# leeyevi/MV3D_TF

Measured on AMD Instinct MI355X. Metric: KITTI-shape frames/sec (RPN+3-view ROI-pool+NMS) at 1/2/4/8 MI355X, higher is better.
Workload: dtype f32

## Files before the change

### include/mv3d_hip.h

```cpp
#ifndef MV3D_HIP_H
#define MV3D_HIP_H
#include <stddef.h>
#include <stdint.h>
#ifdef __cplusplus
extern "C" {
#endif

typedef enum {
    MV3D_OK = 0,
    MV3D_ERR_INVALID_ARG = 1,
    MV3D_ERR_WORKSPACE = 2,
    MV3D_ERR_HIP = 3,
    MV3D_ERR_ZERO_DIVISION = 4
} mv3d_status;

int mv3d_version(void);
const char *mv3d_status_string(int status);


size_t mv3d_nms_workspace_bytes(int max_boxes);
int mv3d_nms_device(const float *dets_dev, int n, double thresh, int max_keep,
                    int32_t *keep_dev, int32_t *num_keep_dev, int32_t *status_dev,
                    void *workspace, size_t workspace_bytes, void *stream);

int mv3d_nms_round_plan(int num_boxes, int max_keep, int32_t *rounds_out);

int mv3d_nms_device_trace(const float *dets_dev, int n, double thresh, int max_keep,
                          int32_t *keep_dev, int32_t *num_keep_dev, int32_t *status_dev,
                          void *workspace, size_t workspace_bytes, void *stream, int64_t *trace_dev);

int mv3d_nms_host(int32_t *keep_out, int32_t *num_out, const float *dets_host, int n,
                  double thresh, int device_id);

void _nms(int *keep_out, int *num_out, const float *boxes_host, int boxes_num,
          int boxes_dim, float nms_overlap_thresh, int device_id);

typedef struct {
    int32_t feat_stride;
    int32_t pre_nms_topN;
    int32_t post_nms_topN;
    int32_t img_height;
    int32_t img_width;
    int32_t img_padding;
    int32_t nms_strict_gt;
    int32_t reserved0;
    double nms_thresh;
    double min_size;
} mv3d_proposal_params;

int mv3d_proposal_3d_capacity(int H, int W, const mv3d_proposal_params *p);
size_t mv3d_proposal_3d_workspace_bytes(int batch, int H, int W, const mv3d_proposal_params *p);
int mv3d_proposal_3d(const float *prob_dev, const float *pred_dev, int batch, int H, int W,
                     const float *im_info_dev, const float *calib_dev,
                     const mv3d_proposal_params *p,
                     float *blob_bv_dev, float *blob_img_dev, float *blob_3d_dev,
                     int32_t *num_out_dev, int32_t *status_dev,
                     void *workspace, size_t workspace_bytes, void *stream);
int mv3d_proposal_3d_masked(const float *prob_dev, const float *pred_dev, int batch, int H, int W,
                            const float *im_info_dev, const float *calib_dev,
                            const mv3d_proposal_params *p, const uint8_t *anchor_mask_dev,
                            float *blob_bv_dev, float *blob_img_dev, float *blob_3d_dev,
                            int32_t *num_out_dev, int32_t *status_dev,
                            void *workspace, size_t workspace_bytes, void *stream);

size_t mv3d_anchor_occupancy_workspace_bytes(int batch, int map_h, int map_w);
int mv3d_anchor_occupancy(const float *bev_dev, int batch, int map_h, int map_w, int channels,
                          int H, int W, int feat_stride, int min_cells,
                          uint8_t *mask_dev, int32_t *count_dev,
                          void *workspace, size_t workspace_bytes, void *stream);

int mv3d_roi_pool_forward(const float *bottom_data, float spatial_scale, int batch_size,
                          int num_rois, int height, int width, int channels,
                          int pooled_height, int pooled_width, const float *bottom_rois,
                          float *top_data, int32_t *argmax_data, void *stream);
int mv3d_roi_pool_backward(const float *top_diff, float spatial_scale, int batch_size,
                           int num_rois, int height, int width, int channels,
                           int pooled_height, int pooled_width, const float *bottom_rois,
                           float *bottom_diff, const int32_t *argmax_data, void *stream);

#define MV3D_MAX_ROI_VIEWS 4
typedef struct {
    const float *bottom_data;
    const float *bottom_rois;
    float *top_data;
    int32_t *argmax_data;
    float spatial_scale;
    int32_t batch_size, num_rois, height, width, channels;
} mv3d_roi_view;
int mv3d_roi_pool_forward_views(int num_views, const mv3d_roi_view *views, int pooled_height, int pooled_width,
                                void *stream);
int mv3d_roi_pool_forward_views_cold(int num_views, const mv3d_roi_view *views, int pooled_height, int pooled_width,
                                     void *stream);
int mv3d_roi_pool_forward_views_half(int num_views, const mv3d_roi_view *views, int pooled_height, int pooled_width,
                                     int top_type, int cold_maps, void *stream);

typedef struct {
    float *bottom_diff;
    const float *bottom_rois;
    const float *top_diff;
    const int32_t *argmax_data;
    float spatial_scale;
    int32_t batch_size, num_rois, height, width, channels;
} mv3d_roi_grad_view;
size_t mv3d_roi_pool_backward_workspace_bytes(int num_views, const mv3d_roi_grad_view *views, int pooled_height,
                                              int pooled_width);
int mv3d_roi_pool_backward_views(int num_views, const mv3d_roi_grad_view *views, int pooled_height, int pooled_width,
                                 void *workspace, size_t workspace_bytes, void *stream);
const char *mv3d_roi_pool_backward_path(int num_views, const mv3d_roi_grad_view *views, int pooled_height, int pooled_width,
                                        int have_workspace, int pair);

size_t mv3d_roi_pool_pair_workspace_bytes(int num_views, const mv3d_roi_grad_view *views, int pooled_height, int pooled_width);
int mv3d_roi_pool_forward_views_pair(int num_views, const mv3d_roi_view *views, int pooled_height, int pooled_width,
                                     int cold_maps, void *stream);
int mv3d_roi_pool_backward_views_pair(int num_views, const mv3d_roi_grad_view *views, int pooled_height, int pooled_width,
                                      void *workspace, size_t workspace_bytes, void *stream);
int mv3d_roi_pool_argmax_decode(int num_views, const mv3d_roi_view *views, int pooled_height, int pooled_width,
                                int32_t *const *argmax_out, void *stream);

int mv3d_ROIPoolForwardLaucher(const float *bottom_data, float spatial_scale, int num_rois, int height, int width, int channels,
                               int pooled_height, int pooled_width, const float *bottom_rois, float *top_data,
                               int32_t *argmax_data, void *stream);
int mv3d_ROIPoolBackwardLaucher(const float *top_diff, float spatial_scale, int batch_size, int num_rois, int height, int width,
                                int channels, int pooled_height, int pooled_width, const float *bottom_rois,
                                float *bottom_diff, const int32_t *argmax_data, void *stream);

int mv3d_rois_3d_to_fv(const float *rois_3d_dev, int num_rois, float *rois_fv_dev, void *stream);

#define MV3D_FV_MAX_FRAMES 1024
size_t mv3d_point_cloud_2_front_workspace(int num_frames);
int mv3d_point_cloud_2_front(const float *points_dev, const int32_t *offsets_dev, int num_frames, int total_points, float *fv_dev,
                             void *workspace_dev, void *stream);

typedef struct {
    int32_t feat_stride;
    int32_t clobber_positives;
    double negative_overlap;
    double positive_overlap;
} mv3d_anchor_target_params;

size_t mv3d_anchor_target_workspace_bytes(int H, int W, int G);
int mv3d_anchor_target_stage1(int H, int W, const float *im_info_dev, const float *gt_bv_dev,
                              const float *gt_3d_dev, int G, const mv3d_anchor_target_params *p,
                              float *labels_dev, float *targets_dev, int32_t *counts_dev,
                              uint8_t *fg_hi_dev, void *workspace, size_t workspace_bytes,
                              void *stream);
int mv3d_anchor_target_stage2(int H, int W, const mv3d_anchor_target_params *p,
                              const int32_t *disable_fg_dev, int n_dis_fg,
                              const int32_t *disable_bg1_dev, int n_dis_bg1,
                              const int32_t *disable_bg2_dev, int n_dis_bg2,
                              float *labels_dev, float *anchors_dev, float *anchors_3d_dev,
                              int32_t *n_anchors_dev, int anchors_cap,
                              void *workspace, size_t workspace_bytes, void *stream);

int mv3d_anchor_target_stage1_batch(int batch, int H, int W, const float *im_info_dev, const float *const *gt_bv_dev,
                                    const float *const *gt_3d_dev, const int *G, const mv3d_anchor_target_params *p,
                                    float *labels_dev, float *targets_dev, int32_t *const *counts_dev,
                                    uint8_t *const *fg_hi_dev, void *const *workspace, size_t workspace_bytes, void *stream);
int mv3d_anchor_target_stage1_batch_masked(int batch, int H, int W, const float *im_info_dev, const float *const *gt_bv_dev,
                                           const float *const *gt_3d_dev, const int *G, const mv3d_anchor_target_params *p,
                                           const uint8_t *const *anchor_mask_dev, float *labels_dev, float *targets_dev,
                                           int32_t *const *counts_dev, uint8_t *const *fg_hi_dev, void *const *workspace,
                                           size_t workspace_bytes, void *stream);
int mv3d_anchor_target_stage2_batch(int batch, int H, int W, const mv3d_anchor_target_params *p,
                                    const int32_t *const *disable_fg_dev, const int *n_dis_fg,
                                    const int32_t *const *disable_bg1_dev, const int *n_dis_bg1,
                                    const int32_t *const *disable_bg2_dev, const int *n_dis_bg2, float *labels_dev,
                                    float *anchors_dev, float *anchors_3d_dev, int32_t *n_anchors_dev, int anchors_cap,
                                    void *const *workspace, size_t workspace_bytes, void *stream);

typedef struct {
    int32_t num_classes;
    int32_t frame_index;
    double fg_thresh;
    double bg_thresh_hi;
    double bg_thresh_lo;
} mv3d_proposal_target_params;

size_t mv3d_proposal_target_workspace_bytes(int num_rois, int G);
int mv3d_proposal_target_stage1(const float *rois_bv_dev, const float *rois_3d_dev, int num_rois,
                                const float *gt_bv_dev, const float *gt_3d_dev, int G,
                                const mv3d_proposal_target_params *p, int32_t *counts_dev,
                                void *workspace, size_t workspace_bytes, void *stream);
int mv3d_proposal_target_stage2(const float *rois_bv_dev, const float *rois_3d_dev, int num_rois,
                                const float *gt_bv_dev, const float *gt_3d_dev,
                                const float *gt_corners_dev, int G, const float *calib_dev,
                                const mv3d_proposal_target_params *p,
                                const int32_t *fg_pick_dev, int n_fg, const int32_t *bg_pick_dev, int n_bg,
                                float *rois_bv_out, float *rois_img_out, int32_t *labels_out,
                                float *bbox_targets_out, float *rois_3d_out,
                                void *workspace, size_t workspace_bytes, void *stream);

int mv3d_proposal_target_stage1_batch(int batch, const float *const *rois_bv_dev, const float *const *rois_3d_dev,
                                      const int *num_rois, const float *const *gt_bv_dev, const float *const *gt_3d_dev,
                                      const int *G, const mv3d_proposal_target_params *params, int32_t *const *counts_dev,
                                      void *const *workspace, const size_t *workspace_bytes, void *stream);
int mv3d_proposal_target_stage2_batch(int batch, const float *const *rois_bv_dev, const float *const *rois_3d_dev,
                                      const int *num_rois, const float *const *gt_bv_dev, const float *const *gt_3d_dev,
                                      const float *const *gt_corners_dev, const int *G, const float *const *calib_dev,
                                      const mv3d_proposal_target_params *params, const int32_t *const *fg_pick_dev,
                                      const int *n_fg, const int32_t *const *bg_pick_dev, const int *n_bg,
                                      float *const *rois_bv_out, float *const *rois_img_out, int32_t *const *labels_out,
                                      float *const *bbox_targets_out, float *const *rois_3d_out, float *const *rois_fv_out,
                                      void *const *workspace, const size_t *workspace_bytes, void *stream);
int mv3d_proposal_target_stage1_batch_devn(int batch, const float *const *rois_bv_dev, const float *const *rois_3d_dev,
                                           const int *num_rois_cap, const int32_t *const *num_rois_dev,
                                           const float *const *gt_bv_dev, const float *const *gt_3d_dev, const int *G,
                                           const mv3d_proposal_target_params *params, int32_t *const *counts_dev,
                                           void *const *workspace, const size_t *workspace_bytes, void *stream);
int mv3d_proposal_target_stage2_batch_devn(int batch, const float *const *rois_bv_dev, const float *const *rois_3d_dev,
                                           const int *num_rois_cap, const int32_t *const *num_rois_dev,
                                           const float *const *gt_bv_dev, const float *const *gt_3d_dev,
                                           const float *const *gt_corners_dev, const int *G, const float *const *calib_dev,
                                           const mv3d_proposal_target_params *params, const int32_t *const *fg_pick_dev,
                                           const int *n_fg, const int32_t *const *bg_pick_dev, const int *n_bg,
                                           float *const *rois_bv_out, float *const *rois_img_out, int32_t *const *labels_out,
                                           float *const *bbox_targets_out, float *const *rois_3d_out, float *const *rois_fv_out,
                                           void *const *workspace, const size_t *workspace_bytes, void *stream);

int mv3d_point_cloud_2_top(const float *points_dev, int num_points, float *top_dev, void *stream);

int mv3d_point_cloud_2_top_shape(double res, double zres, double side_lo, double side_hi, double fwd_lo, double fwd_hi,
                                 double height_lo, double height_hi, int *dims);
int mv3d_point_cloud_2_top_ranges(const float *points_dev, int num_points, double res, double zres, double side_lo, double side_hi,
                                  double fwd_lo, double fwd_hi, double height_lo, double height_hi, float *top_dev,
                                  int *status_dev, void *stream);

int mv3d_point_cloud_2_top_batch(const float *points_dev, const int32_t *offsets_dev, int num_frames, int total_points,
                                 const double *ranges8_host, float *top_dev, int32_t *status_dev, void *stream);
int mv3d_point_cloud_2_top_batch_dense(const float *points_dev, const int32_t *offsets_dev, int num_frames, int total_points,
                                       const double *ranges8_host, float *top_dev, int32_t *status_dev, void *stream);

int mv3d_point_cloud_2_top_paper_batch(const float *points_dev, const int32_t *offsets_dev, int num_frames, int total_points,
                                       const double *ranges8_host, float *top_dev, void *workspace_dev, int32_t *status_dev,
                                       void *stream);
size_t mv3d_point_cloud_2_top_paper_workspace(int num_frames, const double *ranges8_host);
int mv3d_point_cloud_2_top_paper_shape(double res, double zres, double side_lo, double side_hi, double fwd_lo, double fwd_hi,
                                       double height_lo, double height_hi, int *dims);
int mv3d_bev_density_table(float *out64);

size_t mv3d_scan_crop_workspace(int total_points);
int mv3d_scan_crop_tile_rows(void);
int mv3d_scan_crop_to_image(const float *points_dev, const int32_t *offsets_dev, int num_frames, int total_points,
                            const float *calib_dev, const int32_t *image_hw_dev, float *points_out_dev, int32_t *offsets_out_dev,
                            void *workspace_dev, size_t workspace_bytes, void *stream);

int mv3d_scan_transform(const float *points_dev, const int32_t *offsets_dev, int num_frames, int total_points,
                        const double *xform_dev, float *points_out_dev, void *stream);

int mv3d_legacy_permutation(void *mt19937_state, int32_t n, int32_t *out);
typedef struct {
    int32_t n_fg, n_bg, n_low;
    int32_t pt_n_fg, pt_n_bg;
    int32_t reserved0;
    const uint8_t *fg_alive;
} mv3d_draw_frame;
typedef struct {
    int32_t rpn_batchsize;
    int32_t rpn_num_fg;
    int32_t rois_per_image;
    int32_t roi_fg_max;
} mv3d_draw_params;
int mv3d_draw_training_subsamples(void *mt19937_state, int batch, const mv3d_draw_frame *frames, const mv3d_draw_params *par,
                                  int32_t *lists, size_t lists_cap, int32_t *sizes, int32_t *scratch, size_t scratch_cap);

typedef struct {
    int32_t batch, H, W, num_classes;
    int32_t proposal_cap;
    int32_t anchor_cap;
    int32_t roi_cap;
    int32_t max_gt;
    mv3d_proposal_params proposal;
    mv3d_anchor_target_params anchor;
    mv3d_proposal_target_params target;
    mv3d_draw_params draw;
} mv3d_train_path_config;
typedef struct {
    float *blob_bv, *blob_img, *blob_3d;
    int32_t *num_proposals;
    void *proposal_ws; size_t proposal_ws_bytes;
    float *rpn_labels, *rpn_targets;
    float *anchors, *anchors_3d;
    int32_t *n_anchors;
    uint8_t *report; size_t report_row;
    int32_t *pt_counts;
    void *anchor_ws; size_t anchor_ws_bytes;
    void *target_ws; size_t target_ws_bytes;
    float *rois_bev, *rois_rgb, *rois_fv;
    float *rois_3d; int32_t *labels; float *bbox_targets;
    int32_t *lists; size_t lists_cap;
    uint8_t *h_report; size_t h_report_row;
    int32_t *h_pt_counts;
    int32_t *h_num_proposals;
    int32_t *h_lists;
    int32_t *h_scratch; size_t scratch_cap;
} mv3d_train_path_slot;
typedef struct mv3d_train_path mv3d_train_path;
int mv3d_train_path_create(const mv3d_train_path_config *config, int depth, const mv3d_train_path_slot *slots, int helper_thread,
                           mv3d_train_path **out);
int mv3d_train_path_configure(mv3d_train_path *path, const mv3d_train_path_config *config);
int mv3d_train_path_submit(mv3d_train_path *path, int slot, const float *prob_dev, const float *pred_dev, const float *im_info_dev,
                           const float *calib_dev, const float *const *gt_bv_dev, const float *const *gt_3d_dev,
                           const float *const *gt_corners_dev, const int *G, void *mt19937_state, void *stream);
int mv3d_train_path_submit_masked(mv3d_train_path *path, int slot, const float *prob_dev, const float *pred_dev,
                                  const float *im_info_dev, const float *calib_dev, const float *const *gt_bv_dev,
                                  const float *const *gt_3d_dev, const float *const *gt_corners_dev, const int *G,
                                  const uint8_t *anchor_mask_dev, void *mt19937_state, void *stream);
int mv3d_train_path_finish(mv3d_train_path *path, int slot, int32_t *rows_out, int32_t *num_proposals_out, int32_t *sizes_out);
int mv3d_train_path_host_seconds(mv3d_train_path *path, double *wait_s, double *draw_s);
void mv3d_train_path_destroy(mv3d_train_path *path);

int mv3d_gt_encode(const float *box_cam_dev, const double *cos_sin_dev, int num_objects, const float *inv_rot_dev,
                   const float *tr_velo_to_cam_dev, float *corners_cam_dev, float *corners_lidar_dev,
                   float *boxes_3d_dev, float *boxes_bv_dev, void *stream);

int mv3d_box_detect_tail(const float *rois_3d_dev, const float *bbox_pred_dev, int num_rois, int num_classes,
                         float *corners_dev, float *pred_cnr_r_dev, float *pred_bv_dev, float *pred_bv_r_dev,
                         void *stream);

typedef struct {
    int32_t num_classes;
    int32_t rows_per_frame;
    int32_t max_per_image;
    int32_t nms_strict_gt;
    float score_thresh;
    int32_t reserved0;
    double nms_thresh;
} mv3d_detect_post_params;

size_t mv3d_detect_post_workspace_bytes(int batch, const mv3d_detect_post_params *p);
int mv3d_detect_post(const float *cls_prob_dev, const float *pred_bv_dev, const float *corners_dev,
                     const float *pred_cnr_r_dev, const int32_t *num_rois_dev, int batch,
                     const mv3d_detect_post_params *p, float *det_bv_dev, float *det_cnr_dev, float *det_cnr_r_dev,
                     int32_t *det_row_dev, int32_t *det_count_dev, int32_t *status_dev, void *workspace,
                     size_t workspace_bytes, void *stream);

#define MV3D_DETECT_STATUS_NONFINITE 2
size_t mv3d_detect_post_oriented_workspace_bytes(int batch, const mv3d_detect_post_params *p);
int mv3d_detect_post_oriented(const float *cls_prob_dev, const float *pred_bv_dev, const float *corners_dev,
                              const float *pred_cnr_r_dev, const int32_t *num_rois_dev, int batch,
                              const mv3d_detect_post_params *p, int footprint_source, float *det_bv_dev, float *det_cnr_dev,
                              float *det_cnr_r_dev, int32_t *det_row_dev, int32_t *det_count_dev, int32_t *status_dev,
                              void *workspace, size_t workspace_bytes, void *stream);

size_t mv3d_loss_workspace_bytes(int rows);
int mv3d_rpn_loss(const float *rpn_cls_score_dev, const float *rpn_labels_dev, const float *rpn_bbox_pred_dev,
                  const float *rpn_bbox_targets_dev, int num_anchors, float sigma, float *losses_dev,
                  float *d_cls_score_dev, float *d_bbox_pred_dev, void *workspace, size_t workspace_bytes, void *stream);
int mv3d_rcnn_loss(const float *cls_score_dev, const int32_t *labels_dev, const float *bbox_pred_dev,
                   const float *bbox_targets_dev, int num_rois, int num_classes, int box_dim, float sigma,
                   float *losses_dev, float *d_cls_score_dev, float *d_bbox_pred_dev, void *workspace,
                   size_t workspace_bytes, void *stream);
int mv3d_rcnn_loss_ignore(const float *cls_score_dev, const int32_t *labels_dev, const float *bbox_pred_dev,
                          const float *bbox_targets_dev, int num_rois, int num_classes, int box_dim, float sigma,
                          float *losses_dev, float *d_cls_score_dev, float *d_bbox_pred_dev, void *workspace,
                          size_t workspace_bytes, void *stream);

int mv3d_ignore_relabel(const float *rpn_labels_dev, const int32_t *roi_labels_dev, const float *rois_bv_dev,
                        const float *rois_img_dev, int num_rois, const float *calib_dev, int batch, int H, int W,
                        int feat_stride, const float *ignore_bv_dev, const int32_t *ignore_bv_off_dev, int ignore_bv_rows,
                        const float *ignore_img_dev, const int32_t *ignore_img_off_dev, int ignore_img_rows, double overlap,
                        float *rpn_labels_out_dev, int32_t *roi_labels_out_dev, int32_t *counts_dev, int32_t *status_dev,
                        void *stream);

int mv3d_conv3x3_f16(const void *x_framed, const void *w_packed, const float *bias, void *y, int batch, int height, int width,
                     int c_in, int c_out, int out_framed, int out_f32, int relu, void *stream);
int mv3d_conv3x3_f32(const void *x_framed, const void *w_packed, const float *bias, void *y, int batch, int height, int width, int c_in,
                     int c_out, int out_framed, int relu, void *stream);
int mv3d_maxpool2x2_f32(const void *x_framed, void *y_framed, int batch, int height, int width, int channels, void *stream);
int mv3d_frame_nhwc_f32(const float *x_nhwc, void *y_framed, int batch, int height, int width, int channels, int channels_out,
                        void *stream);
int mv3d_conv3x3_bf16(const void *x_framed, const void *w_packed, const float *bias, void *y, int batch, int height, int width,
                      int c_in, int c_out, int out_framed, int out_f32, int relu, void *stream);
int mv3d_conv3x3_gated_bf16(const void *x_framed, const void *w_packed, const float *bias, const void *gate_framed, void *y,
                            int batch, int height, int width, int c_in, int c_out, void *stream);
int mv3d_maxpool2x2_bf16(const void *x_framed, void *y_framed, int batch, int height, int width, int channels, void *stream);
int mv3d_frame_nhwc_bf16(const float *x_nhwc, void *y_framed, int batch, int height, int width, int channels, int channels_out,
                         void *stream);
int mv3d_maxpool2x2_bwd_bf16(const void *y_framed, const void *g_pooled_framed, void *gy_framed, int batch, int height, int width,
                             int channels, void *stream);
int mv3d_maxpool2x2_bwd_f32(const void *y_framed, const void *g_pooled_framed, void *gy_framed, int batch, int height, int width,
                            int channels, void *stream);
#define MV3D_MAX_CONV_VIEWS 3
typedef struct {
    const void *x_framed;
    const void *w_packed;
    const float *bias;
    const void *gate_framed;
    void *y;
    int32_t batch, height, width, reserved0;
} mv3d_conv_view;
int mv3d_conv3x3_views_f16(int num_views, const mv3d_conv_view *views, int c_in, int c_out, int out_framed, int out_f32, int relu,
                           void *stream);
int mv3d_conv3x3_views_bf16(int num_views, const mv3d_conv_view *views, int c_in, int c_out, int out_framed, int out_f32, int relu,
                            void *stream);
int mv3d_conv3x3_views_f32(int num_views, const mv3d_conv_view *views, int c_in, int c_out, int out_framed, int relu, void *stream);
int mv3d_conv3x3_pool_views_f16(int num_views, const mv3d_conv_view *views, int c_in, int c_out, void *stream);
int mv3d_conv3x3_pool_views_bf16(int num_views, const mv3d_conv_view *views, int c_in, int c_out, void *stream);
const char *mv3d_conv3x3_path(int operand_bytes, int num_views, const int32_t *pixels, int c_in, int c_out, int out_f32, int gated,
                              int pool);
typedef struct {
    const void *x_framed;
    const void *g_pooled_framed;
    void *y_framed;
    int32_t batch, height, width, reserved0;
} mv3d_pool_view;
int mv3d_maxpool2x2_views_f16(int num_views, const mv3d_pool_view *views, int channels, void *stream);
int mv3d_maxpool2x2_views_bf16(int num_views, const mv3d_pool_view *views, int channels, void *stream);
int mv3d_maxpool2x2_views_f32(int num_views, const mv3d_pool_view *views, int channels, void *stream);
int mv3d_maxpool2x2_bwd_views_bf16(int num_views, const mv3d_pool_view *views, int channels, void *stream);
int mv3d_maxpool2x2_bwd_views_f32(int num_views, const mv3d_pool_view *views, int channels, void *stream);
size_t mv3d_conv3x3_wgrad_workspace_bytes(int batch, int height, int width, int c_in, int c_out);
int mv3d_conv3x3_wgrad_bf16(const void *x_framed, const void *dy_framed, float *dw, float *db, int batch, int height, int width,
                            int c_in, int c_in_real, int c_out, void *workspace, size_t workspace_bytes, void *stream);
size_t mv3d_conv3x3_wgrad_f32_workspace_bytes(int batch, int height, int width, int c_in, int c_out);
int mv3d_conv3x3_wgrad_f32(const void *x_framed, const void *dy_framed, float *dw, float *db, int batch, int height, int width,
                           int c_in, int c_in_real, int c_out, void *workspace, size_t workspace_bytes, void *stream);
typedef struct {
    const void *x_framed;
    const void *dy_framed;
    float *dw;
    float *db;
    int32_t batch, height, width;
    int32_t c_in_real;
} mv3d_wgrad_view;
size_t mv3d_conv3x3_wgrad_views_workspace_bytes(int num_views, const mv3d_wgrad_view *views, int c_in, int c_out, int f32_maps);
int mv3d_conv3x3_wgrad_views_bf16(int num_views, const mv3d_wgrad_view *views, int c_in, int c_in_real, int c_out, void *workspace,
                                  size_t workspace_bytes, void *stream);
int mv3d_conv3x3_wgrad_views_f32(int num_views, const mv3d_wgrad_view *views, int c_in, int c_in_real, int c_out, void *workspace,
                                 size_t workspace_bytes, void *stream);
int mv3d_conv3x3_pack_bf16(const float *w_oihw, void *fwd_packed, void *dgrad_packed, int c_out, int c_in, int c_in_pad, void *stream);
typedef struct {
    const float *w_oihw;
    void *fwd_packed, *dgrad_packed;
    int32_t c_out, c_in, c_in_pad, reserved0;
} mv3d_pack_item;
int mv3d_conv3x3_pack_many_bf16(int num_items, const mv3d_pack_item *items, void *stream);
int mv3d_conv3x3_pack_many_f32(int num_items, const mv3d_pack_item *items, void *stream);
int mv3d_maxpool2x2_f16(const void *x_framed, void *y_framed, int batch, int height, int width, int channels, void *stream);
int mv3d_frame_nhwc_f16(const float *x_nhwc, void *y_framed, int batch, int height, int width, int channels, int channels_out,
                        void *stream);

int mv3d_softmax_rows(const float *logits_dev, float *prob_dev, long long rows, int classes, void *stream);

typedef struct {
    float *param;
    const float *grad;
    float *exp_avg, *exp_avg_sq;
    long long numel;
    void *param_lowp;
} mv3d_adam_tensor;
int mv3d_adam_chunk_elements(void);
int mv3d_adam_step(const mv3d_adam_tensor *tensors_dev, const int32_t *chunk_tensor_dev, const int32_t *chunk_first_dev, int num_chunks,
                   double lr, double beta1, double beta2, double eps, int step, int lowp_dtype ,
                   void *stream);

#define MV3D_KITTI_MAX_DETS 2048
#define MV3D_KITTI_NUM_SAMPLE_PTS 41
typedef struct {
    int32_t num_frames, num_dets, num_gts, img_height;
    const int32_t *det_off, *gt_off;
    const int32_t *offsets_dev;
    const float *det_cnr_dev, *det_score_dev, *calib_dev, *gt_cnr_dev;
    const int32_t *gt_cls_dev;
    const float *gt_attr_dev;
} mv3d_kitti_split;
int mv3d_kitti_eval_overlaps(const mv3d_kitti_split *split, long long num_pairs, double *iou_dev, double *det_height_dev,
                             void *stream);
int mv3d_kitti_eval_match(const mv3d_kitti_split *split, long long num_pairs, const double *iou_dev, const double *det_height_dev,
                          int eval_class, int neighbor_class, double min_overlap, float *matched_dev, void *stream);
int mv3d_kitti_eval_count(const mv3d_kitti_split *split, long long num_pairs, const double *iou_dev, const double *det_height_dev,
                          int eval_class, int neighbor_class, double min_overlap, const float *thresholds_dev,
                          const int32_t *num_thresholds_dev, int32_t *counts_dev, void *stream);

typedef struct {
    int32_t num_dontcare, reserved0;
    const int32_t *dc_off;
    const int32_t *dc_off_dev;
    const float *gt_box_dev, *gt_alpha_dev, *dc_box_dev;
    const int32_t *image_shape_dev;
} mv3d_kitti_image_split;
int mv3d_kitti_eval_image_boxes(const mv3d_kitti_split *split, const mv3d_kitti_image_split *image, double *det_box_dev,
                                double *det_cam_dev, void *stream);
int mv3d_kitti_eval_match_2d(const mv3d_kitti_split *split, const mv3d_kitti_image_split *image, const double *det_box_dev,
                             int eval_class, int neighbor_class, double min_overlap, float *matched_dev, void *stream);
int mv3d_kitti_eval_count_2d(const mv3d_kitti_split *split, const mv3d_kitti_image_split *image, const double *det_box_dev,
                             const double *det_cam_dev, int eval_class, int neighbor_class, double min_overlap,
                             const float *thresholds_dev, const int32_t *num_thresholds_dev, int32_t *counts_dev,
                             double *similarity_dev, void *stream);

#define MV3D_RECALL_MAX_GT 256
#define MV3D_RECALL_SHORT_ASSERT 0
#define MV3D_RECALL_SHORT_ZERO 1
#define MV3D_RECALL_STATUS_SHORT 1
#define MV3D_RECALL_STATUS_NONFINITE 2
typedef struct {
    int32_t num_frames, num_gts, num_limits, num_thresholds, short_mode, reserved0;
    long long num_boxes;
    const int32_t *box_off, *gt_off;
    const int32_t *box_off_dev, *gt_off_dev;
    const float *boxes_dev, *gt_dev;
    const int32_t *limits_dev;
    const double *thresholds_dev;
} mv3d_recall_split;
int mv3d_proposal_recall(const mv3d_recall_split *split, double *gt_overlaps_dev, int32_t *counts_dev, int32_t *status_dev,
                         void *stream);

#define MV3D_RECALL3D_BOX6 0
#define MV3D_RECALL3D_CNR24 1
typedef struct {
    int32_t num_frames, num_gts, num_limits, num_thresholds, short_mode, box_format;
    long long num_boxes, num_pairs;
    const int32_t *box_off, *gt_off, *pair_off;
    const int32_t *box_off_dev, *gt_off_dev, *pair_off_dev;
    const float *boxes_dev, *gt_cnr_dev;
    const int32_t *limits_dev;
    const double *thresholds_dev;
} mv3d_recall3d_split;
size_t mv3d_proposal_recall_3d_workspace_bytes(long long num_pairs);
int mv3d_proposal_recall_3d(const mv3d_recall3d_split *split, double *iou_ws_dev, double *gt_overlaps_dev, int32_t *counts_dev,
                            int32_t *status_dev, void *stream);
int mv3d_proposal_recall_3d_overlaps(const mv3d_recall3d_split *split, double *iou_ws_dev, int32_t *status_dev, void *stream);
int mv3d_proposal_recall_3d_match(const mv3d_recall3d_split *split, const double *iou_ws_dev, double *gt_overlaps_dev,
                                  int32_t *counts_dev, int32_t *status_dev, void *stream);

int mv3d_mirror_columns(float *data_dev, long long rows, int width, int channels, void *stream);

#define MV3D_IMAGE_MAX_FRAMES 1024
int mv3d_image_blob(const uint8_t *pixels_dev, int total_bytes, const int32_t *frames_dev, int num_frames, const double *means3_host,
                    int canvas_h, int canvas_w, float *out_dev, void *stream);

int mv3d_fusion_join_forward(const void *h_dev, int dtype, int sets_in, int paths, int views, int rows, int channels,
                             const uint8_t *keep, const uint8_t *drop_dev, float scale, void *out_dev, void *stream);
int mv3d_fusion_join_backward(const void *h_dev, const void *g_out_dev, int dtype, int sets_in, int paths, int views, int rows,
                              int channels, const uint8_t *keep, const uint8_t *drop_dev, float scale, void *g_h_dev, void *stream);

typedef struct {
    const void *in;
    void *out;
    int64_t frame_stride, row_stride, pixel_stride;
    int32_t dtype, batch, height, width, channels, factor;
} mv3d_upsample_view;
int mv3d_upsample_bilinear_views(int num_views, const mv3d_upsample_view *views, void *stream);
int mv3d_upsample_bilinear_backward_views(int num_views, const mv3d_upsample_view *views, void *stream);

#ifdef __cplusplus
}
#endif
#endif
```

### mv3d_tf_amd/_lib.py

```python
import ctypes as C
import os

import torch

_HERE = os.path.dirname(os.path.abspath(__file__))
LIB_PATH = os.path.join(_HERE, "libmv3d_hip.so")

OK, ERR_INVALID_ARG, ERR_WORKSPACE, ERR_HIP, ERR_ZERO_DIVISION = 0, 1, 2, 3, 4
MAX_ROI_VIEWS = 4


class ProposalParams(C.Structure):
    _fields_ = [("feat_stride", C.c_int32), ("pre_nms_topN", C.c_int32), ("post_nms_topN", C.c_int32),
                ("img_height", C.c_int32), ("img_width", C.c_int32), ("img_padding", C.c_int32),
                ("nms_strict_gt", C.c_int32), ("reserved0", C.c_int32), ("nms_thresh", C.c_double), ("min_size", C.c_double)]


class DetectPostParams(C.Structure):
    _fields_ = [("num_classes", C.c_int32), ("rows_per_frame", C.c_int32), ("max_per_image", C.c_int32),
                ("nms_strict_gt", C.c_int32), ("score_thresh", C.c_float), ("reserved0", C.c_int32), ("nms_thresh", C.c_double)]


class AnchorTargetParams(C.Structure):
    _fields_ = [("feat_stride", C.c_int32), ("clobber_positives", C.c_int32),
                ("negative_overlap", C.c_double), ("positive_overlap", C.c_double)]


class RoiView(C.Structure):
    _fields_ = [("bottom_data", C.c_void_p), ("bottom_rois", C.c_void_p), ("top_data", C.c_void_p),
                ("argmax_data", C.c_void_p), ("spatial_scale", C.c_float), ("batch_size", C.c_int32),
                ("num_rois", C.c_int32), ("height", C.c_int32), ("width", C.c_int32), ("channels", C.c_int32)]


class RoiGradView(C.Structure):
    _fields_ = [("bottom_diff", C.c_void_p), ("bottom_rois", C.c_void_p), ("top_diff", C.c_void_p),
                ("argmax_data", C.c_void_p), ("spatial_scale", C.c_float), ("batch_size", C.c_int32),
                ("num_rois", C.c_int32), ("height", C.c_int32), ("width", C.c_int32), ("channels", C.c_int32)]


class ProposalTargetParams(C.Structure):
    _fields_ = [("num_classes", C.c_int32), ("frame_index", C.c_int32), ("fg_thresh", C.c_double),
                ("bg_thresh_hi", C.c_double), ("bg_thresh_lo", C.c_double)]


class DrawFrame(C.Structure):
    _fields_ = [("n_fg", C.c_int32), ("n_bg", C.c_int32), ("n_low", C.c_int32), ("pt_n_fg", C.c_int32), ("pt_n_bg", C.c_int32),
                ("reserved0", C.c_int32), ("fg_alive", C.c_void_p)]


class DrawParams(C.Structure):
    _fields_ = [("rpn_batchsize", C.c_int32), ("rpn_num_fg", C.c_int32), ("rois_per_image", C.c_int32), ("roi_fg_max", C.c_int32)]


class TrainPathConfig(C.Structure):
    _fields_ = [("batch", C.c_int32), ("H", C.c_int32), ("W", C.c_int32), ("num_classes", C.c_int32), ("proposal_cap", C.c_int32),
                ("anchor_cap", C.c_int32), ("roi_cap", C.c_int32), ("max_gt", C.c_int32), ("proposal", ProposalParams),
                ("anchor", AnchorTargetParams), ("target", ProposalTargetParams), ("draw", DrawParams)]


class TrainPathSlot(C.Structure):
    _fields_ = [("blob_bv", C.c_void_p), ("blob_img", C.c_void_p), ("blob_3d", C.c_void_p), ("num_proposals", C.c_void_p),
                ("proposal_ws", C.c_void_p), ("proposal_ws_bytes", C.c_size_t), ("rpn_labels", C.c_void_p), ("rpn_targets", C.c_void_p),
                ("anchors", C.c_void_p), ("anchors_3d", C.c_void_p), ("n_anchors", C.c_void_p), ("report", C.c_void_p),
                ("report_row", C.c_size_t), ("pt_counts", C.c_void_p), ("anchor_ws", C.c_void_p), ("anchor_ws_bytes", C.c_size_t),
                ("target_ws", C.c_void_p), ("target_ws_bytes", C.c_size_t), ("rois_bev", C.c_void_p), ("rois_rgb", C.c_void_p),
                ("rois_fv", C.c_void_p), ("rois_3d", C.c_void_p), ("labels", C.c_void_p), ("bbox_targets", C.c_void_p),
                ("lists", C.c_void_p), ("lists_cap", C.c_size_t), ("h_report", C.c_void_p), ("h_report_row", C.c_size_t),
                ("h_pt_counts", C.c_void_p), ("h_num_proposals", C.c_void_p), ("h_lists", C.c_void_p), ("h_scratch", C.c_void_p),
                ("scratch_cap", C.c_size_t)]


class ConvView(C.Structure):
    _fields_ = [("x_framed", C.c_void_p), ("w_packed", C.c_void_p), ("bias", C.c_void_p), ("gate_framed", C.c_void_p), ("y", C.c_void_p),
                ("batch", C.c_int32), ("height", C.c_int32), ("width", C.c_int32), ("reserved0", C.c_int32)]


class PoolView(C.Structure):
    _fields_ = [("x_framed", C.c_void_p), ("g_pooled_framed", C.c_void_p), ("y_framed", C.c_void_p),
                ("batch", C.c_int32), ("height", C.c_int32), ("width", C.c_int32), ("reserved0", C.c_int32)]


class WgradView(C.Structure):
    _fields_ = [("x_framed", C.c_void_p), ("dy_framed", C.c_void_p), ("dw", C.c_void_p), ("db", C.c_void_p),
                ("batch", C.c_int32), ("height", C.c_int32), ("width", C.c_int32), ("c_in_real", C.c_int32)]


class PackItem(C.Structure):
    _fields_ = [("w_oihw", C.c_void_p), ("fwd_packed", C.c_void_p), ("dgrad_packed", C.c_void_p),
                ("c_out", C.c_int32), ("c_in", C.c_int32), ("c_in_pad", C.c_int32), ("reserved0", C.c_int32)]


class AdamTensor(C.Structure):
    _fields_ = [("param", C.c_void_p), ("grad", C.c_void_p), ("exp_avg", C.c_void_p), ("exp_avg_sq", C.c_void_p), ("numel", C.c_longlong),
                ("param_lowp", C.c_void_p)]


class KittiSplit(C.Structure):
    _fields_ = [("num_frames", C.c_int32), ("num_dets", C.c_int32), ("num_gts", C.c_int32), ("img_height", C.c_int32),
                ("det_off", C.c_void_p), ("gt_off", C.c_void_p), ("offsets_dev", C.c_void_p), ("det_cnr_dev", C.c_void_p),
                ("det_score_dev", C.c_void_p), ("calib_dev", C.c_void_p), ("gt_cnr_dev", C.c_void_p), ("gt_cls_dev", C.c_void_p),
                ("gt_attr_dev", C.c_void_p)]


class KittiImageSplit(C.Structure):
    _fields_ = [("num_dontcare", C.c_int32), ("reserved0", C.c_int32), ("dc_off", C.c_void_p), ("dc_off_dev", C.c_void_p),
                ("gt_box_dev", C.c_void_p), ("gt_alpha_dev", C.c_void_p), ("dc_box_dev", C.c_void_p), ("image_shape_dev", C.c_void_p)]


class RecallSplit(C.Structure):
    _fields_ = [("num_frames", C.c_int32), ("num_gts", C.c_int32), ("num_limits", C.c_int32), ("num_thresholds", C.c_int32),
                ("short_mode", C.c_int32), ("reserved0", C.c_int32), ("num_boxes", C.c_longlong), ("box_off", C.c_void_p),
                ("gt_off", C.c_void_p), ("box_off_dev", C.c_void_p), ("gt_off_dev", C.c_void_p), ("boxes_dev", C.c_void_p),
                ("gt_dev", C.c_void_p), ("limits_dev", C.c_void_p), ("thresholds_dev", C.c_void_p)]


class Recall3dSplit(C.Structure):
    _fields_ = [("num_frames", C.c_int32), ("num_gts", C.c_int32), ("num_limits", C.c_int32), ("num_thresholds", C.c_int32),
                ("short_mode", C.c_int32), ("box_format", C.c_int32), ("num_boxes", C.c_longlong), ("num_pairs", C.c_longlong),
                ("box_off", C.c_void_p), ("gt_off", C.c_void_p), ("pair_off", C.c_void_p), ("box_off_dev", C.c_void_p),
                ("gt_off_dev", C.c_void_p), ("pair_off_dev", C.c_void_p), ("boxes_dev", C.c_void_p), ("gt_cnr_dev", C.c_void_p),
                ("limits_dev", C.c_void_p), ("thresholds_dev", C.c_void_p)]


class UpsampleView(C.Structure):
    _fields_ = [("in_", C.c_void_p), ("out", C.c_void_p), ("frame_stride", C.c_int64), ("row_stride", C.c_int64),
                ("pixel_stride", C.c_int64), ("dtype", C.c_int32), ("batch", C.c_int32), ("height", C.c_int32), ("width", C.c_int32),
                ("channels", C.c_int32), ("factor", C.c_int32)]


_P = C.c_void_p
_SIGS = {
    "mv3d_version": (C.c_int, []),
    "mv3d_status_string": (C.c_char_p, [C.c_int]),
    "mv3d_nms_workspace_bytes": (C.c_size_t, [C.c_int]),
    "mv3d_nms_round_plan": (C.c_int, [C.c_int, C.c_int, C.POINTER(C.c_int32)]),
    "mv3d_nms_device": (C.c_int, [_P, C.c_int, C.c_double, C.c_int, _P, _P, _P, _P, C.c_size_t, _P]),
    "mv3d_nms_device_trace": (C.c_int, [_P, C.c_int, C.c_double, C.c_int, _P, _P, _P, _P, C.c_size_t, _P, _P]),
    "mv3d_nms_host": (C.c_int, [_P, _P, _P, C.c_int, C.c_double, C.c_int]),
    "_nms": (None, [_P, _P, _P, C.c_int, C.c_int, C.c_float, C.c_int]),
    "mv3d_proposal_3d_capacity": (C.c_int, [C.c_int, C.c_int, C.POINTER(ProposalParams)]),
    "mv3d_proposal_3d_workspace_bytes": (C.c_size_t, [C.c_int, C.c_int, C.c_int, C.POINTER(ProposalParams)]),
    "mv3d_proposal_3d": (C.c_int, [_P, _P, C.c_int, C.c_int, C.c_int, _P, _P, C.POINTER(ProposalParams),
                                   _P, _P, _P, _P, _P, _P, C.c_size_t, _P]),
    "mv3d_proposal_3d_masked": (C.c_int, [_P, _P, C.c_int, C.c_int, C.c_int, _P, _P, C.POINTER(ProposalParams),
                                          _P, _P, _P, _P, _P, _P, _P, C.c_size_t, _P]),
    "mv3d_anchor_occupancy_workspace_bytes": (C.c_size_t, [C.c_int, C.c_int, C.c_int]),
    "mv3d_anchor_occupancy": (C.c_int, [_P, C.c_int, C.c_int, C.c_int, C.c_int, C.c_int, C.c_int, C.c_int, C.c_int, _P, _P, _P,
                                        C.c_size_t, _P]),
    "mv3d_roi_pool_forward": (C.c_int, [_P, C.c_float, C.c_int, C.c_int, C.c_int, C.c_int, C.c_int, C.c_int,
                                        C.c_int, _P, _P, _P, _P]),
    "mv3d_roi_pool_backward": (C.c_int, [_P, C.c_float, C.c_int, C.c_int, C.c_int, C.c_int, C.c_int, C.c_int,
                                         C.c_int, _P, _P, _P, _P]),
    "mv3d_anchor_target_workspace_bytes": (C.c_size_t, [C.c_int, C.c_int, C.c_int]),
    "mv3d_anchor_target_stage1": (C.c_int, [C.c_int, C.c_int, _P, _P, _P, C.c_int, C.POINTER(AnchorTargetParams),
                                            _P, _P, _P, _P, _P, C.c_size_t, _P]),
    "mv3d_anchor_target_stage2": (C.c_int, [C.c_int, C.c_int, C.POINTER(AnchorTargetParams), _P, C.c_int, _P,
                                            C.c_int, _P, C.c_int, _P, _P, _P, _P, C.c_int, _P, C.c_size_t, _P]),
    "mv3d_anchor_target_stage1_batch": (C.c_int, [C.c_int, C.c_int, C.c_int, _P, _P, _P, _P, C.POINTER(AnchorTargetParams), _P, _P, _P, _P,
                                                  _P, C.c_size_t, _P]),
    "mv3d_anchor_target_stage1_batch_masked": (C.c_int, [C.c_int, C.c_int, C.c_int, _P, _P, _P, _P, C.POINTER(AnchorTargetParams), _P, _P,
                                                         _P, _P, _P, _P, C.c_size_t, _P]),
    "mv3d_anchor_target_stage2_batch": (C.c_int, [C.c_int, C.c_int, C.c_int, C.POINTER(AnchorTargetParams), _P, _P, _P, _P, _P, _P, _P,
                                                  _P, _P, _P, C.c_int, _P, C.c_size_t, _P]),
    "mv3d_proposal_target_stage1_batch": (C.c_int, [C.c_int, _P, _P, _P, _P, _P, _P, _P, _P, _P, _P, _P]),
    "mv3d_proposal_target_stage2_batch": (C.c_int, [C.c_int, _P, _P, _P, _P, _P, _P, _P, _P, _P, _P, _P, _P, _P, _P, _P, _P, _P, _P, _P,
                                                    _P, _P, _P]),
    "mv3d_proposal_target_stage1_batch_devn": (C.c_int, [C.c_int, _P, _P, _P, _P, _P, _P, _P, _P, _P, _P, _P, _P]),
    "mv3d_proposal_target_stage2_batch_devn": (C.c_int, [C.c_int, _P, _P, _P, _P, _P, _P, _P, _P, _P, _P, _P, _P, _P, _P, _P, _P, _P, _P,
                                                         _P, _P, _P, _P, _P]),
    "mv3d_proposal_target_workspace_bytes": (C.c_size_t, [C.c_int, C.c_int]),
    "mv3d_proposal_target_stage1": (C.c_int, [_P, _P, C.c_int, _P, _P, C.c_int, C.POINTER(ProposalTargetParams), _P, _P,
                                              C.c_size_t, _P]),
    "mv3d_proposal_target_stage2": (C.c_int, [_P, _P, C.c_int, _P, _P, _P, C.c_int, _P, C.POINTER(ProposalTargetParams),
                                              _P, C.c_int, _P, C.c_int, _P, _P, _P, _P, _P, _P, C.c_size_t, _P]),
    "mv3d_point_cloud_2_top": (C.c_int, [_P, C.c_int, _P, _P]),
    "mv3d_point_cloud_2_top_shape": (C.c_int, [C.c_double] * 8 + [_P]),
    "mv3d_point_cloud_2_top_ranges": (C.c_int, [_P, C.c_int] + [C.c_double] * 8 + [_P, _P, _P]),
    "mv3d_point_cloud_2_top_batch": (C.c_int, [_P, _P, C.c_int, C.c_int, _P, _P, _P, _P]),
    "mv3d_point_cloud_2_top_batch_dense": (C.c_int, [_P, _P, C.c_int, C.c_int, _P, _P, _P, _P]),
    "mv3d_point_cloud_2_top_paper_batch": (C.c_int, [_P, _P, C.c_int, C.c_int, _P, _P, _P, _P, _P]),
    "mv3d_point_cloud_2_top_paper_workspace": (C.c_size_t, [C.c_int, _P]),
    "mv3d_point_cloud_2_top_paper_shape": (C.c_int, [C.c_double] * 8 + [_P]),
    "mv3d_bev_density_table": (C.c_int, [_P]),
    "mv3d_scan_crop_workspace": (C.c_size_t, [C.c_int]),
    "mv3d_scan_crop_tile_rows": (C.c_int, []),
    "mv3d_scan_crop_to_image": (C.c_int, [_P, _P, C.c_int, C.c_int, _P, _P, _P, _P, _P, C.c_size_t, _P]),
    "mv3d_scan_transform": (C.c_int, [_P, _P, C.c_int, C.c_int, _P, _P, _P]),
    "mv3d_box_detect_tail": (C.c_int, [_P, _P, C.c_int, C.c_int, _P, _P, _P, _P, _P]),
    "mv3d_detect_post_workspace_bytes": (C.c_size_t, [C.c_int, C.POINTER(DetectPostParams)]),
    "mv3d_detect_post": (C.c_int, [_P, _P, _P, _P, _P, C.c_int, C.POINTER(DetectPostParams), _P, _P, _P, _P, _P, _P, _P, C.c_size_t,
                                   _P]),
    "mv3d_detect_post_oriented_workspace_bytes": (C.c_size_t, [C.c_int, C.POINTER(DetectPostParams)]),
    "mv3d_detect_post_oriented": (C.c_int, [_P, _P, _P, _P, _P, C.c_int, C.POINTER(DetectPostParams), C.c_int, _P, _P, _P, _P, _P, _P,
                                            _P, C.c_size_t, _P]),
    "mv3d_loss_workspace_bytes": (C.c_size_t, [C.c_int]),
    "mv3d_rpn_loss": (C.c_int, [_P, _P, _P, _P, C.c_int, C.c_float, _P, _P, _P, _P, C.c_size_t, _P]),
    "mv3d_rcnn_loss": (C.c_int, [_P, _P, _P, _P, C.c_int, C.c_int, C.c_int, C.c_float, _P, _P, _P, _P, C.c_size_t, _P]),
    "mv3d_rcnn_loss_ignore": (C.c_int, [_P, _P, _P, _P, C.c_int, C.c_int, C.c_int, C.c_float, _P, _P, _P, _P, C.c_size_t, _P]),
    "mv3d_ignore_relabel": (C.c_int, [_P, _P, _P, _P, C.c_int, _P, C.c_int, C.c_int, C.c_int, C.c_int, _P, _P, C.c_int, _P, _P, C.c_int,
                                      C.c_double, _P, _P, _P, _P, _P]),
    "mv3d_roi_pool_forward_views": (C.c_int, [C.c_int, C.POINTER(RoiView), C.c_int, C.c_int, _P]),
    "mv3d_roi_pool_forward_views_cold": (C.c_int, [C.c_int, C.POINTER(RoiView), C.c_int, C.c_int, _P]),
    "mv3d_roi_pool_forward_views_half": (C.c_int, [C.c_int, C.POINTER(RoiView), C.c_int, C.c_int, C.c_int, C.c_int, _P]),
    "mv3d_roi_pool_backward_workspace_bytes": (C.c_size_t, [C.c_int, C.POINTER(RoiGradView), C.c_int, C.c_int]),
    "mv3d_roi_pool_backward_views": (C.c_int, [C.c_int, C.POINTER(RoiGradView), C.c_int, C.c_int, _P, C.c_size_t, _P]),
    "mv3d_roi_pool_backward_path": (C.c_char_p, [C.c_int, C.POINTER(RoiGradView), C.c_int, C.c_int, C.c_int, C.c_int]),
    "mv3d_roi_pool_pair_workspace_bytes": (C.c_size_t, [C.c_int, C.POINTER(RoiGradView), C.c_int, C.c_int]),
    "mv3d_roi_pool_forward_views_pair": (C.c_int, [C.c_int, C.POINTER(RoiView), C.c_int, C.c_int, C.c_int, _P]),
    "mv3d_roi_pool_backward_views_pair": (C.c_int, [C.c_int, C.POINTER(RoiGradView), C.c_int, C.c_int, _P, C.c_size_t, _P]),
    "mv3d_roi_pool_argmax_decode": (C.c_int, [C.c_int, C.POINTER(RoiView), C.c_int, C.c_int, C.POINTER(C.c_void_p), _P]),
    "mv3d_ROIPoolForwardLaucher": (C.c_int, [_P, C.c_float, C.c_int, C.c_int, C.c_int, C.c_int, C.c_int, C.c_int, _P, _P, _P, _P]),
    "mv3d_ROIPoolBackwardLaucher": (C.c_int, [_P, C.c_float, C.c_int, C.c_int, C.c_int, C.c_int, C.c_int, C.c_int, C.c_int, _P, _P, _P, _P]),
    "mv3d_rois_3d_to_fv": (C.c_int, [_P, C.c_int, _P, _P]),
    "mv3d_point_cloud_2_front_workspace": (C.c_size_t, [C.c_int]),
    "mv3d_point_cloud_2_front": (C.c_int, [_P, _P, C.c_int, C.c_int, _P, _P, _P]),
    "mv3d_legacy_permutation": (C.c_int, [_P, C.c_int32, _P]),
    "mv3d_draw_training_subsamples": (C.c_int, [_P, C.c_int, C.POINTER(DrawFrame), C.POINTER(DrawParams), _P, C.c_size_t, _P, _P,
                                                C.c_size_t]),
    "mv3d_train_path_create": (C.c_int, [C.POINTER(TrainPathConfig), C.c_int, C.POINTER(TrainPathSlot), C.c_int, C.POINTER(C.c_void_p)]),
    "mv3d_train_path_configure": (C.c_int, [_P, C.POINTER(TrainPathConfig)]),
    "mv3d_train_path_submit": (C.c_int, [_P, C.c_int, _P, _P, _P, _P, _P, _P, _P, _P, _P, _P]),
    "mv3d_train_path_submit_masked": (C.c_int, [_P, C.c_int, _P, _P, _P, _P, _P, _P, _P, _P, _P, _P, _P]),
    "mv3d_train_path_finish": (C.c_int, [_P, C.c_int, _P, _P, _P]),
    "mv3d_train_path_host_seconds": (C.c_int, [_P, C.POINTER(C.c_double), C.POINTER(C.c_double)]),
    "mv3d_train_path_destroy": (None, [_P]),
    "mv3d_gt_encode": (C.c_int, [_P, _P, C.c_int, _P, _P, _P, _P, _P, _P, _P]),
    "mv3d_conv3x3_f16": (C.c_int, [_P, _P, _P, _P, C.c_int, C.c_int, C.c_int, C.c_int, C.c_int, C.c_int, C.c_int, C.c_int, _P]),
    "mv3d_conv3x3_f32": (C.c_int, [_P, _P, _P, _P, C.c_int, C.c_int, C.c_int, C.c_int, C.c_int, C.c_int, C.c_int, _P]),
    "mv3d_maxpool2x2_f32": (C.c_int, [_P, _P, C.c_int, C.c_int, C.c_int, C.c_int, _P]),
    "mv3d_frame_nhwc_f32": (C.c_int, [_P, _P, C.c_int, C.c_int, C.c_int, C.c_int, C.c_int, _P]),
    "mv3d_conv3x3_bf16": (C.c_int, [_P, _P, _P, _P, C.c_int, C.c_int, C.c_int, C.c_int, C.c_int, C.c_int, C.c_int, C.c_int, _P]),
    "mv3d_maxpool2x2_bf16": (C.c_int, [_P, _P, C.c_int, C.c_int, C.c_int, C.c_int, _P]),
    "mv3d_frame_nhwc_bf16": (C.c_int, [_P, _P, C.c_int, C.c_int, C.c_int, C.c_int, C.c_int, _P]),
    "mv3d_conv3x3_wgrad_workspace_bytes": (C.c_size_t, [C.c_int, C.c_int, C.c_int, C.c_int, C.c_int]),
    "mv3d_conv3x3_wgrad_bf16": (C.c_int, [_P, _P, _P, _P, C.c_int, C.c_int, C.c_int, C.c_int, C.c_int, C.c_int, _P, C.c_size_t, _P]),
    "mv3d_conv3x3_wgrad_f32_workspace_bytes": (C.c_size_t, [C.c_int, C.c_int, C.c_int, C.c_int, C.c_int]),
    "mv3d_conv3x3_wgrad_f32": (C.c_int, [_P, _P, _P, _P, C.c_int, C.c_int, C.c_int, C.c_int, C.c_int, C.c_int, _P, C.c_size_t, _P]),
    "mv3d_conv3x3_pack_bf16": (C.c_int, [_P, _P, _P, C.c_int, C.c_int, C.c_int, _P]),
    "mv3d_conv3x3_gated_bf16": (C.c_int, [_P, _P, _P, _P, _P, C.c_int, C.c_int, C.c_int, C.c_int, C.c_int, _P]),
    "mv3d_maxpool2x2_bwd_f32": (C.c_int, [_P, _P, _P, C.c_int, C.c_int, C.c_int, C.c_int, _P]),
    "mv3d_maxpool2x2_bwd_bf16": (C.c_int, [_P, _P, _P, C.c_int, C.c_int, C.c_int, C.c_int, _P]),
    "mv3d_conv3x3_views_f16": (C.c_int, [C.c_int, C.POINTER(ConvView), C.c_int, C.c_int, C.c_int, C.c_int, C.c_int, _P]),
    "mv3d_conv3x3_views_bf16": (C.c_int, [C.c_int, C.POINTER(ConvView), C.c_int, C.c_int, C.c_int, C.c_int, C.c_int, _P]),
    "mv3d_conv3x3_views_f32": (C.c_int, [C.c_int, C.POINTER(ConvView), C.c_int, C.c_int, C.c_int, C.c_int, _P]),
    "mv3d_conv3x3_pool_views_f16": (C.c_int, [C.c_int, C.POINTER(ConvView), C.c_int, C.c_int, _P]),
    "mv3d_conv3x3_pool_views_bf16": (C.c_int, [C.c_int, C.POINTER(ConvView), C.c_int, C.c_int, _P]),
    "mv3d_conv3x3_path": (C.c_char_p, [C.c_int, C.c_int, C.POINTER(C.c_int32), C.c_int, C.c_int, C.c_int, C.c_int, C.c_int]),
    "mv3d_maxpool2x2_views_f16": (C.c_int, [C.c_int, C.POINTER(PoolView), C.c_int, _P]),
    "mv3d_maxpool2x2_views_bf16": (C.c_int, [C.c_int, C.POINTER(PoolView), C.c_int, _P]),
    "mv3d_maxpool2x2_views_f32": (C.c_int, [C.c_int, C.POINTER(PoolView), C.c_int, _P]),
    "mv3d_maxpool2x2_bwd_views_bf16": (C.c_int, [C.c_int, C.POINTER(PoolView), C.c_int, _P]),
    "mv3d_maxpool2x2_bwd_views_f32": (C.c_int, [C.c_int, C.POINTER(PoolView), C.c_int, _P]),
    "mv3d_conv3x3_wgrad_views_workspace_bytes": (C.c_size_t, [C.c_int, C.POINTER(WgradView), C.c_int, C.c_int, C.c_int]),
    "mv3d_conv3x3_wgrad_views_bf16": (C.c_int, [C.c_int, C.POINTER(WgradView), C.c_int, C.c_int, C.c_int, _P, C.c_size_t, _P]),
    "mv3d_conv3x3_wgrad_views_f32": (C.c_int, [C.c_int, C.POINTER(WgradView), C.c_int, C.c_int, C.c_int, _P, C.c_size_t, _P]),
    "mv3d_conv3x3_pack_many_bf16": (C.c_int, [C.c_int, C.POINTER(PackItem), _P]),
    "mv3d_conv3x3_pack_many_f32": (C.c_int, [C.c_int, C.POINTER(PackItem), _P]),
    "mv3d_maxpool2x2_f16": (C.c_int, [_P, _P, C.c_int, C.c_int, C.c_int, C.c_int, _P]),
    "mv3d_frame_nhwc_f16": (C.c_int, [_P, _P, C.c_int, C.c_int, C.c_int, C.c_int, C.c_int, _P]),
    "mv3d_softmax_rows": (C.c_int, [_P, _P, C.c_longlong, C.c_int, _P]),
    "mv3d_adam_chunk_elements": (C.c_int, []),
    "mv3d_adam_step": (C.c_int, [_P, _P, _P, C.c_int, C.c_double, C.c_double, C.c_double, C.c_double, C.c_int, C.c_int, _P]),
    "mv3d_kitti_eval_overlaps": (C.c_int, [C.POINTER(KittiSplit), C.c_longlong, _P, _P, _P]),
    "mv3d_kitti_eval_match": (C.c_int, [C.POINTER(KittiSplit), C.c_longlong, _P, _P, C.c_int, C.c_int, C.c_double, _P, _P]),
    "mv3d_kitti_eval_count": (C.c_int, [C.POINTER(KittiSplit), C.c_longlong, _P, _P, C.c_int, C.c_int, C.c_double, _P, _P, _P, _P]),
    "mv3d_kitti_eval_image_boxes": (C.c_int, [C.POINTER(KittiSplit), C.POINTER(KittiImageSplit), _P, _P, _P]),
    "mv3d_kitti_eval_match_2d": (C.c_int, [C.POINTER(KittiSplit), C.POINTER(KittiImageSplit), _P, C.c_int, C.c_int, C.c_double, _P,
                                           _P]),
    "mv3d_kitti_eval_count_2d": (C.c_int, [C.POINTER(KittiSplit), C.POINTER(KittiImageSplit), _P, _P, C.c_int, C.c_int, C.c_double,
                                           _P, _P, _P, _P, _P]),
    "mv3d_proposal_recall": (C.c_int, [C.POINTER(RecallSplit), _P, _P, _P, _P]),
    "mv3d_proposal_recall_3d_workspace_bytes": (C.c_size_t, [C.c_longlong]),
    "mv3d_proposal_recall_3d": (C.c_int, [C.POINTER(Recall3dSplit), _P, _P, _P, _P, _P]),
    "mv3d_proposal_recall_3d_overlaps": (C.c_int, [C.POINTER(Recall3dSplit), _P, _P, _P]),
    "mv3d_proposal_recall_3d_match": (C.c_int, [C.POINTER(Recall3dSplit), _P, _P, _P, _P, _P]),
    "mv3d_mirror_columns": (C.c_int, [_P, C.c_longlong, C.c_int, C.c_int, _P]),
    "mv3d_image_blob": (C.c_int, [_P, C.c_int, _P, C.c_int, C.POINTER(C.c_double), C.c_int, C.c_int, _P, _P]),
    "mv3d_fusion_join_forward": (C.c_int, [_P, C.c_int, C.c_int, C.c_int, C.c_int, C.c_int, C.c_int, _P, _P, C.c_float, _P, _P]),
    "mv3d_fusion_join_backward": (C.c_int, [_P, _P, C.c_int, C.c_int, C.c_int, C.c_int, C.c_int, C.c_int, _P, _P, C.c_float, _P, _P]),
    "mv3d_upsample_bilinear_views": (C.c_int, [C.c_int, C.POINTER(UpsampleView), _P]),
    "mv3d_upsample_bilinear_backward_views": (C.c_int, [C.c_int, C.POINTER(UpsampleView), _P]),
}
EXPORTS = tuple(_SIGS)

_lib = None


def lib():
    global _lib
    if _lib is None:
        if not os.path.exists(LIB_PATH):
            raise RuntimeError(
                f"{LIB_PATH} is missing: the HIP extension is the product and has no fallback. "
                "Build it with `python -m mv3d_tf_amd.build` (or __graft_entry__.build()).")
        handle = C.CDLL(LIB_PATH)
        for name, (res, args) in _SIGS.items():
            fn = getattr(handle, name)
            fn.restype = res
            fn.argtypes = args
        _lib = handle
    return _lib


class Mv3dError(RuntimeError):
    def __init__(self, status, where):
        self.status = status
        super().__init__(f"{where}: {lib().mv3d_status_string(status).decode()} (status {status})")


def check(status, where):
    if status == ERR_ZERO_DIVISION:
        raise ZeroDivisionError("float division")
    if status != OK:
        raise Mv3dError(status, where)
```

### mv3d_tf_amd/csrc/anchor_target.hip

```cpp
#include <math.h>
#include "geometry.h"

__device__ __forceinline__ double mv3d_log(double x)
{
    if (x != x || x < 0) return NAN;
    if (x == 0) return -INFINITY;
    if (isinf(x)) return x;
    int k;
    double m = frexp(x, &k);
    if (m < 0.70710678118654752440) { m *= 2.0; k -= 1; }
    const double s = (m - 1.0) / (m + 1.0);
    const double z = s * s;
    double p = 1.0 / 39;
#pragma unroll
    for (int d = 37; d >= 1; d -= 2) p = fma(p, z, 1.0 / d);
    const double LN2_HI = 6.93147180369123816490e-01, LN2_LO = 1.90821492927058770002e-10;
    const double lm = 2.0 * s * p;
    return fma((double)k, LN2_HI, fma((double)k, LN2_LO, lm));
}

struct AtDev {
    int H, W, N, G, stride, clobber;
    double neg_ov, pos_ov;
    const float *im_info, *gt_bv, *gt_3d;
    const uint8_t *mask;
    double *max_ov;
    int32_t *argmax;
    unsigned long long *gtpart;
    int nblk;
    float *labels, *targets;
};

#define AT_MAX_BATCH 16
struct AtLists {
    int32_t *fg, *bg, *low;
};
struct AtFrame {
    AtDev d;
    AtLists lists;
    int32_t *counts;
    uint8_t *fg_hi;
    int32_t *agg1, *agg2;
    const int32_t *dis_fg, *dis_bg1, *dis_bg2;
    int n_dis_fg, n_dis_bg1, n_dis_bg2;
    float *anchors, *anchors_3d;
    int32_t *n_anchors;
};
struct AtBatch { AtFrame f[AT_MAX_BATCH]; int cap, n_agg1, n_agg2; };

__device__ __forceinline__ bool anchor_box(const AtDev &d, int n, int &x1, int &y1, int &x2, int &y2)
{
    grid_anchor(n, d.W, d.stride, x1, y1, x2, y2);
    return x1 >= 0 && y1 >= 0 && (double)x2 < (double)d.im_info[1] && (double)y2 < (double)d.im_info[0] && (!d.mask || d.mask[n]);
}

__global__ __launch_bounds__(256) void at_overlap_kernel(AtBatch bt)
{
    const AtDev &d = bt.f[blockIdx.y].d;
    if (blockIdx.x == 0) {
        const AtFrame &F = bt.f[blockIdx.y];
        for (int t = threadIdx.x; t < bt.n_agg1; t += blockDim.x) F.agg1[t] = 0;
        for (int t = threadIdx.x; t < bt.n_agg2; t += blockDim.x) F.agg2[t] = 0;
    }
    __shared__ float s_gt[TARGET_MAX_GT * 4];
    __shared__ unsigned long long s_max[TARGET_MAX_GT];
    stage_gt_bv(d.gt_bv, d.G, s_gt);
    for (int g = threadIdx.x; g < d.G; g += blockDim.x) s_max[g] = 0ull;
    __syncthreads();
    const int n = blockIdx.x * blockDim.x + threadIdx.x;
    if (n < d.N) {
        int x1, y1, x2, y2;
        const bool inside = anchor_box(d, n, x1, y1, x2, y2);
        double mx = -1.0;
        int am = 0;
        if (inside) {
            for (int g = 0; g < d.G; ++g) {
                const double o = bbox_overlap_f64(x1, y1, x2, y2, s_gt[4 * g], s_gt[4 * g + 1], s_gt[4 * g + 2], s_gt[4 * g + 3]);
                if (o > mx) { mx = o; am = g; }
                if (o > 0.0) atomicMax(&s_max[g], (unsigned long long)__double_as_longlong(o));
            }
        }
        d.max_ov[n] = mx;
        d.argmax[n] = am;
    }
    __syncthreads();
    for (int g = threadIdx.x; g < d.G; g += blockDim.x) d.gtpart[(long long)g * d.nblk + blockIdx.x] = s_max[g];
}

__global__ __launch_bounds__(256) void at_label_kernel(AtBatch bt)
{
    const AtDev &d = bt.f[blockIdx.y].d;
    __shared__ float s_gt[TARGET_MAX_GT * 4];
    __shared__ unsigned long long s_maxu[TARGET_MAX_GT];
    stage_gt_bv(d.gt_bv, d.G, s_gt);
    for (int g = threadIdx.x; g < d.G; g += blockDim.x) s_maxu[g] = 0ull;
    __syncthreads();
    for (int i = threadIdx.x; i < d.G * d.nblk; i += blockDim.x) {
        const unsigned long long v = d.gtpart[i];
        if (v) atomicMax(&s_maxu[i / d.nblk], v);
    }
    __syncthreads();
    const double *s_max = reinterpret_cast<const double *>(s_maxu);
    const int n = blockIdx.x * blockDim.x + threadIdx.x;
    if (n >= d.N) return;
    int x1, y1, x2, y2;
    const bool inside = anchor_box(d, n, x1, y1, x2, y2);
    float lab = -1.0f;
    float T[6] = {0, 0, 0, 0, 0, 0};
    if (inside) {
        const double mx = d.max_ov[n];
        if (!d.clobber && 0 < mx && mx < d.neg_ov) lab = 0.0f;
        for (int g = 0; g < d.G; ++g) {
            const double o = bbox_overlap_f64(x1, y1, x2, y2, s_gt[4 * g], s_gt[4 * g + 1], s_gt[4 * g + 2], s_gt[4 * g + 3]);
            if (o == s_max[g]) { lab = 1.0f; break; }
        }
        if (mx >= d.pos_ov) lab = 1.0f;
        if (d.clobber && mx < d.neg_ov) lab = 0.0f;
        if (d.G > 0) {
            double A[6];
            anchor_to_lidar_f64(x1, y1, x2, y2, A);
            const double ex = A[0], ey = A[1], ez = A[2], ex_len = A[3], ex_wid = A[4], eh = A[5];
            const float *gt = d.gt_3d + 7 * d.argmax[n];
            T[0] = (float)(((double)gt[0] - ex) / ex_wid);
            T[1] = (float)(((double)gt[1] - ey) / ex_len);
            T[2] = (float)(((double)gt[2] - ez) / eh);
            T[3] = (float)mv3d_log((double)gt[3] / ex_len);
            T[4] = (float)mv3d_log((double)gt[4] / ex_wid);
            T[5] = (float)mv3d_log((double)gt[5] / eh);
        }
    }
    d.labels[n] = lab;
#pragma unroll
    for (int j = 0; j < 6; ++j) d.targets[6 * (long long)n + j] = T[j];
}

__global__ __launch_bounds__(256) void at_compact_kernel(AtBatch bt)
{
    const AtFrame &F = bt.f[blockIdx.y];
    const float *labels = F.d.labels;
    const double *max_ov = F.d.max_ov;
    const double neg_ov = F.d.neg_ov;
    const AtLists L = F.lists;
    uint8_t *fg_hi = F.fg_hi;
    int tot[4];
    mv3d_grid_compact<4>(
        F.d.N,
        [&](int n, bool f[4]) {
            const double mx = max_ov[n];
            const float lab = labels[n];
            const bool inside = (mx >= 0.0);
            f[0] = inside; f[1] = inside && (lab == 1.0f); f[2] = inside && (lab == 0.0f); f[3] = inside && (mx < neg_ov);
        },
        [&](int k, int pos, int n) {
            if (k == 1) { L.fg[pos] = n; fg_hi[pos] = (max_ov[n] >= neg_ov) ? 1 : 0; }
            else if (k == 2) L.bg[pos] = n;
            else if (k == 3) L.low[pos] = n;
        },
        F.agg1, tot);
    if (blockIdx.x == gridDim.x - 1 && threadIdx.x == 0) {
        int32_t *counts = F.counts;
        counts[0] = tot[0]; counts[1] = tot[1]; counts[2] = tot[2]; counts[3] = tot[3];
        counts[4] = counts[5] = counts[6] = counts[7] = 0;
    }
}

__global__ __launch_bounds__(256) void at_disable_all_kernel(AtBatch bt)
{
    const AtFrame &F = bt.f[blockIdx.y];
    const int n1 = F.n_dis_fg, n2 = F.n_dis_bg1, n3 = F.n_dis_bg2;
    for (int t = blockIdx.x * blockDim.x + threadIdx.x; t < n1 + n2 + n3; t += gridDim.x * blockDim.x) {
        if (t < n1) F.d.labels[F.lists.fg[F.dis_fg[t]]] = -1.0f;
        else if (t < n1 + n2) F.d.labels[F.lists.bg[F.dis_bg1[t - n1]]] = -1.0f;
        else F.d.argmax[F.lists.low[F.dis_bg2[t - n1 - n2]]] = -1;
    }
}

__global__ __launch_bounds__(256) void at_emit_relabel_kernel(AtBatch bt)
{
    const AtFrame &F = bt.f[blockIdx.y];
    const AtDev &d = F.d;
    float *anchors = F.anchors, *anchors_3d = F.anchors_3d;
    const int cap = bt.cap;
    int tot[1];
    mv3d_grid_compact<1>(
        d.N,
        [&](int n, bool f[1]) { f[0] = anchors && (d.max_ov[n] >= 0.0) && (d.labels[n] != -1.0f); },
        [&](int, int r, int n) {
            if (r >= cap) return;
            int x1, y1, x2, y2;
            grid_anchor(n, d.W, d.stride, x1, y1, x2, y2);
            float *A = anchors + 5 * (long long)r, *B = anchors_3d + 7 * (long long)r;
            A[0] = 0.0f; A[1] = (float)x1; A[2] = (float)y1; A[3] = (float)x2; A[4] = (float)y2;
            B[0] = 0.0f;
            anchor_to_lidar(x1, y1, x2, y2, B + 1);
        },
        F.agg2, tot);
    if (blockIdx.x == gridDim.x - 1 && threadIdx.x == 0 && F.n_anchors) F.n_anchors[0] = tot[0];
    const int lane = threadIdx.x & 63, wave = threadIdx.x >> 6;
    const int beg = blockIdx.x * MV3D_GC_ITEMS + wave * 256;
#pragma unroll
    for (int u = 0; u < 4; ++u) {
        const int n = beg + 64 * u + lane;
        if (n < d.N) {
            const double mx = d.max_ov[n];
            if (mx >= 0.0 && mx < d.neg_ov) d.labels[n] = (d.argmax[n] < 0) ? -1.0f : 0.0f;
        }
    }
}

struct AtLayout { size_t o_maxov, o_argmax, o_gtpart, o_agg1, o_agg2, o_fg, o_bg, o_low, total; int N, ncwg, nblk; };

static bool at_layout(int H, int W, int G, AtLayout &L)
{
    if (H <= 0 || W <= 0 || G < 0 || G > TARGET_MAX_GT) return false;
    const long long N = (long long)H * W * 4;
    if (N > (1 << 22)) return false;
    L.N = (int)N;
    size_t o = 0;
    L.o_maxov = o; o += mv3d_align_up((size_t)N * 8);
    L.o_argmax = o; o += mv3d_align_up((size_t)N * 4);
    L.nblk = (int)((N + 255) / 256);
    L.ncwg = (int)((N + MV3D_GC_ITEMS - 1) / MV3D_GC_ITEMS);
    L.o_agg1 = o; o += mv3d_align_up((size_t)(L.ncwg * 4 + 1) * 4);
    L.o_agg2 = o; o += mv3d_align_up((size_t)(L.ncwg * 1 + 1) * 4);
    L.o_fg = o; o += mv3d_align_up((size_t)N * 4);
    L.o_bg = o; o += mv3d_align_up((size_t)N * 4);
    L.o_low = o; o += mv3d_align_up((size_t)N * 4);
    L.o_gtpart = o; o += mv3d_align_up((size_t)(G > 0 ? G : 1) * L.nblk * 8);
    L.total = o;
    return true;
}

extern "C" size_t mv3d_anchor_target_workspace_bytes(int H, int W, int G)
{
    AtLayout L;
    return at_layout(H, W, G, L) ? L.total : 0;
}

static void at_fill(AtDev &d, const AtLayout &L, int H, int W, int G, const mv3d_anchor_target_params *p, char *ws)
{
    d.H = H; d.W = W; d.N = L.N; d.G = G; d.stride = p->feat_stride; d.clobber = p->clobber_positives;
    d.neg_ov = p->negative_overlap; d.pos_ov = p->positive_overlap;
    d.max_ov = (double *)(ws + L.o_maxov); d.argmax = (int32_t *)(ws + L.o_argmax);
    d.gtpart = (unsigned long long *)(ws + L.o_gtpart); d.nblk = L.nblk;
}

static void at_frame(AtFrame &F, const AtLayout &L, int H, int W, int G, const mv3d_anchor_target_params *p, char *ws)
{
    at_fill(F.d, L, H, W, G, p, ws);
    F.lists.fg = (int32_t *)(ws + L.o_fg); F.lists.bg = (int32_t *)(ws + L.o_bg); F.lists.low = (int32_t *)(ws + L.o_low);
    F.agg1 = (int32_t *)(ws + L.o_agg1); F.agg2 = (int32_t *)(ws + L.o_agg2);
}

extern "C" int mv3d_anchor_target_stage1_batch_masked(int batch, int H, int W, const float *im_info_dev,
                                                      const float *const *gt_bv_dev, const float *const *gt_3d_dev, const int *G,
                                                      const mv3d_anchor_target_params *p, const uint8_t *const *anchor_mask_dev,
                                                      float *labels_dev, float *targets_dev, int32_t *const *counts_dev,
                                                      uint8_t *const *fg_hi_dev, void *const *workspace, size_t workspace_bytes,
                                                      void *stream)
{
    if (batch <= 0 || batch > AT_MAX_BATCH || !p || p->feat_stride <= 0 || !im_info_dev || !labels_dev || !targets_dev ||
        !gt_bv_dev || !gt_3d_dev || !G || !counts_dev || !fg_hi_dev || !workspace)
        return MV3D_ERR_INVALID_ARG;
    hipStream_t s = (hipStream_t)stream;
    AtBatch bt = {};
    AtLayout L = {};
    for (int b = 0; b < batch; ++b) {
        if (!at_layout(H, W, G[b], L)) return MV3D_ERR_INVALID_ARG;
        if (!counts_dev[b] || !fg_hi_dev[b] || (G[b] > 0 && (!gt_bv_dev[b] || !gt_3d_dev[b]))) return MV3D_ERR_INVALID_ARG;
        if (!workspace[b] || workspace_bytes < L.total || ((uintptr_t)workspace[b] % MV3D_ALIGN)) return MV3D_ERR_WORKSPACE;
        AtFrame &F = bt.f[b];
        at_frame(F, L, H, W, G[b], p, (char *)workspace[b]);
        F.d.im_info = im_info_dev + 3 * b; F.d.gt_bv = gt_bv_dev[b]; F.d.gt_3d = gt_3d_dev[b];
        F.d.mask = anchor_mask_dev ? anchor_mask_dev[b] : nullptr;
        F.d.labels = labels_dev + (size_t)b * L.N; F.d.targets = targets_dev + (size_t)b * L.N * 6;
        F.counts = counts_dev[b]; F.fg_hi = fg_hi_dev[b];
    }
    bt.n_agg1 = L.ncwg * 4 + 1; bt.n_agg2 = L.ncwg * 1 + 1;
    const int blocks = L.nblk;
    hipLaunchKernelGGL(at_overlap_kernel, dim3(blocks, batch), dim3(256), 0, s, bt);
    hipLaunchKernelGGL(at_label_kernel, dim3(blocks, batch), dim3(256), 0, s, bt);
    hipLaunchKernelGGL(at_compact_kernel, dim3(L.ncwg, batch), dim3(256), 0, s, bt);
    return mv3d_launch_status();
}

extern "C" int mv3d_anchor_target_stage1_batch(int batch, int H, int W, const float *im_info_dev, const float *const *gt_bv_dev,
                                               const float *const *gt_3d_dev, const int *G, const mv3d_anchor_target_params *p,
                                               float *labels_dev, float *targets_dev, int32_t *const *counts_dev,
                                               uint8_t *const *fg_hi_dev, void *const *workspace, size_t workspace_bytes,
                                               void *stream)
{
    return mv3d_anchor_target_stage1_batch_masked(batch, H, W, im_info_dev, gt_bv_dev, gt_3d_dev, G, p, nullptr, labels_dev, targets_dev,
                                                  counts_dev, fg_hi_dev, workspace, workspace_bytes, stream);
}

extern "C" int mv3d_anchor_target_stage1(int H, int W, const float *im_info_dev, const float *gt_bv_dev,
                                         const float *gt_3d_dev, int G, const mv3d_anchor_target_params *p,
                                         float *labels_dev, float *targets_dev, int32_t *counts_dev, uint8_t *fg_hi_dev,
                                         void *workspace, size_t workspace_bytes, void *stream)
{
    return mv3d_anchor_target_stage1_batch(1, H, W, im_info_dev, &gt_bv_dev, &gt_3d_dev, &G, p, labels_dev, targets_dev,
                                           &counts_dev, &fg_hi_dev, &workspace, workspace_bytes, stream);
}

extern "C" int mv3d_anchor_target_stage2_batch(int batch, int H, int W, const mv3d_anchor_target_params *p,
                                               const int32_t *const *disable_fg_dev, const int *n_dis_fg,
                                               const int32_t *const *disable_bg1_dev, const int *n_dis_bg1,
                                               const int32_t *const *disable_bg2_dev, const int *n_dis_bg2, float *labels_dev,
                                               float *anchors_dev, float *anchors_3d_dev, int32_t *n_anchors_dev,
                                               int anchors_cap, void *const *workspace, size_t workspace_bytes, void *stream)
{
    if (batch <= 0 || batch > AT_MAX_BATCH || !p || !labels_dev || !workspace || !n_dis_fg || !n_dis_bg1 || !n_dis_bg2 ||
        !disable_fg_dev || !disable_bg1_dev || !disable_bg2_dev)
        return MV3D_ERR_INVALID_ARG;
    AtLayout L;
    if (!at_layout(H, W, 0, L)) return MV3D_ERR_INVALID_ARG;
    const bool emit = anchors_dev && anchors_3d_dev && n_anchors_dev;
    AtBatch bt = {};
    bt.cap = anchors_cap;
    int most = 0;
    for (int b = 0; b < batch; ++b) {
        if (n_dis_fg[b] < 0 || n_dis_bg1[b] < 0 || n_dis_bg2[b] < 0) return MV3D_ERR_INVALID_ARG;
        if ((n_dis_fg[b] && !disable_fg_dev[b]) || (n_dis_bg1[b] && !disable_bg1_dev[b]) || (n_dis_bg2[b] && !disable_bg2_dev[b]))
            return MV3D_ERR_INVALID_ARG;
        if (!workspace[b] || workspace_bytes < L.total || ((uintptr_t)workspace[b] % MV3D_ALIGN)) return MV3D_ERR_WORKSPACE;
        AtFrame &F = bt.f[b];
        at_frame(F, L, H, W, 0, p, (char *)workspace[b]);
        F.d.im_info = nullptr; F.d.gt_bv = nullptr; F.d.gt_3d = nullptr; F.d.mask = nullptr; F.d.targets = nullptr;
        F.d.labels = labels_dev + (size_t)b * L.N;
        F.dis_fg = disable_fg_dev[b]; F.dis_bg1 = disable_bg1_dev[b]; F.dis_bg2 = disable_bg2_dev[b];
        F.n_dis_fg = n_dis_fg[b]; F.n_dis_bg1 = n_dis_bg1[b]; F.n_dis_bg2 = n_dis_bg2[b];
        F.anchors = emit ? anchors_dev + (size_t)b * anchors_cap * 5 : nullptr;
        F.anchors_3d = emit ? anchors_3d_dev + (size_t)b * anchors_cap * 7 : nullptr;
        F.n_anchors = emit ? n_anchors_dev + b : nullptr;
        const int n = n_dis_fg[b] + n_dis_bg1[b] + n_dis_bg2[b];
        if (n > most) most = n;
    }
    hipStream_t s = (hipStream_t)stream;
    if (most > 0) hipLaunchKernelGGL(at_disable_all_kernel, dim3((most + 255) / 256, batch), dim3(256), 0, s, bt);
    hipLaunchKernelGGL(at_emit_relabel_kernel, dim3(L.ncwg, batch), dim3(256), 0, s, bt);
    return mv3d_launch_status();
}

extern "C" int mv3d_anchor_target_stage2(int H, int W, const mv3d_anchor_target_params *p,
                                         const int32_t *disable_fg_dev, int n_dis_fg, const int32_t *disable_bg1_dev,
                                         int n_dis_bg1, const int32_t *disable_bg2_dev, int n_dis_bg2, float *labels_dev,
                                         float *anchors_dev, float *anchors_3d_dev, int32_t *n_anchors_dev,
                                         int anchors_cap, void *workspace, size_t workspace_bytes, void *stream)
{
    return mv3d_anchor_target_stage2_batch(1, H, W, p, &disable_fg_dev, &n_dis_fg, &disable_bg1_dev, &n_dis_bg1, &disable_bg2_dev,
                                           &n_dis_bg2, labels_dev, anchors_dev, anchors_3d_dev, n_anchors_dev, anchors_cap,
                                           &workspace, workspace_bytes, stream);
}
```

### mv3d_tf_amd/csrc/legacy_rng.hip

```cpp
#include <stdint.h>
#include <string.h>
#include "../../include/mv3d_hip.h"

namespace {

constexpr int MT_N = 624, MT_M = 397;
struct MtState { uint32_t key[MT_N]; int pos; };

inline void mt_gen(MtState *s)
{
    uint32_t *k = s->key;
    int i;
    for (i = 0; i < MT_N - MT_M; ++i) {
        const uint32_t y = (k[i] & 0x80000000u) | (k[i + 1] & 0x7fffffffu);
        k[i] = k[i + MT_M] ^ (y >> 1) ^ ((y & 1u) ? 0x9908b0dfu : 0u);
    }
    for (; i < MT_N - 1; ++i) {
        const uint32_t y = (k[i] & 0x80000000u) | (k[i + 1] & 0x7fffffffu);
        k[i] = k[i + (MT_M - MT_N)] ^ (y >> 1) ^ ((y & 1u) ? 0x9908b0dfu : 0u);
    }
    const uint32_t y = (k[MT_N - 1] & 0x80000000u) | (k[0] & 0x7fffffffu);
    k[MT_N - 1] = k[MT_M - 1] ^ (y >> 1) ^ ((y & 1u) ? 0x9908b0dfu : 0u);
    s->pos = 0;
}

inline uint32_t mt_next(MtState *s)
{
    if (s->pos == MT_N) mt_gen(s);
    uint32_t y = s->key[s->pos++];
    y ^= (y >> 11);
    y ^= (y << 7) & 0x9d2c5680u;
    y ^= (y << 15) & 0xefc60000u;
    y ^= (y >> 18);
    return y;
}

void permutation(MtState *s, int32_t n, int32_t *x)
{
    for (int32_t i = 0; i < n; ++i) x[i] = i;
    int32_t i = n - 1;
    int pos = s->pos;
    uint32_t t[MT_N];
    int t_lo = MT_N;
    while (i >= 1) {
        const uint32_t mask = 0xffffffffu >> __builtin_clz((uint32_t)i);
        const int32_t lo = (int32_t)(mask >> 1);
        while (i > lo) {
            if (pos == MT_N) { mt_gen(s); pos = 0; t_lo = MT_N; }
            if (t_lo > pos) {
                for (int k = pos; k < MT_N; ++k) {
                    uint32_t y = s->key[k];
                    y ^= (y >> 11);
                    y ^= (y << 7) & 0x9d2c5680u;
                    y ^= (y << 15) & 0xefc60000u;
                    y ^= (y >> 18);
                    t[k] = y;
                }
                t_lo = pos;
            }
            while (pos < MT_N && i > lo) {
                const uint32_t j = t[pos++] & mask;
                const bool ok = j <= (uint32_t)i;
                const uint32_t jj = ok ? j : (uint32_t)i;
                const int32_t a = x[i], b = x[jj];
                x[i] = b; x[jj] = a;
                i -= ok ? 1 : 0;
            }
        }
    }
    s->pos = pos;
}

}

extern "C" int mv3d_legacy_permutation(void *mt19937_state, int32_t n, int32_t *out)
{
    if (!mt19937_state || n < 0 || (n > 0 && !out)) return MV3D_ERR_INVALID_ARG;
    MtState *s = (MtState *)mt19937_state;
    if (s->pos < 0 || s->pos > MT_N) return MV3D_ERR_INVALID_ARG;
    permutation(s, n, out);
    return MV3D_OK;
}

extern "C" int mv3d_draw_training_subsamples(void *mt19937_state, int batch, const mv3d_draw_frame *frames,
                                             const mv3d_draw_params *par, int32_t *lists, size_t lists_cap, int32_t *sizes,
                                             int32_t *scratch, size_t scratch_cap)
{
    if (!mt19937_state || batch <= 0 || !frames || !par || !lists || !sizes || !scratch) return MV3D_ERR_INVALID_ARG;
    MtState *s = (MtState *)mt19937_state;
    if (s->pos < 0 || s->pos > MT_N) return MV3D_ERR_INVALID_ARG;
    size_t o = 0;
    auto emit = [&](int32_t n, int32_t take, bool draw, int32_t *size_out) -> bool {
        *size_out = 0;
        if (!draw) return true;
        if (n < 0 || (size_t)n > scratch_cap || take < 0 || take > n || o + (size_t)take > lists_cap) return false;
        if (take == n) {
            permutation(s, n, lists + o);
        } else {
            permutation(s, n, scratch);
            memcpy(lists + o, scratch, (size_t)take * sizeof(int32_t));
        }
        *size_out = take;
        o += (size_t)take;
        return true;
    };
    for (int b = 0; b < batch; ++b) {
        const mv3d_draw_frame &f = frames[b];
        int32_t *sz = sizes + 5 * b;
        if (f.n_fg < 0 || f.n_bg < 0 || f.n_low < 0 || f.pt_n_fg < 0 || f.pt_n_bg < 0 || (f.n_fg > 0 && !f.fg_alive))
            return MV3D_ERR_INVALID_ARG;
        const int32_t num_fg = par->rpn_num_fg;
        const int32_t *dis_fg = lists + o;
        if (!emit(f.n_fg, f.n_fg - num_fg, f.n_fg > num_fg, &sz[0])) return MV3D_ERR_WORKSPACE;
        const int32_t num_bg = par->rpn_batchsize - (f.n_fg < num_fg ? f.n_fg : num_fg);
        if (!emit(f.n_bg, f.n_bg - num_bg, f.n_bg > num_bg, &sz[1])) return MV3D_ERR_WORKSPACE;
        int32_t n_pos = 0;
        if (f.n_fg > 0) {
            if ((size_t)f.n_fg > scratch_cap) return MV3D_ERR_WORKSPACE;
            uint8_t *alive = (uint8_t *)scratch;
            for (int32_t i = 0; i < f.n_fg; ++i) alive[i] = f.fg_alive[i] ? 1 : 0;
            for (int32_t i = 0; i < sz[0]; ++i) alive[dis_fg[i]] = 0;
            for (int32_t i = 0; i < f.n_fg; ++i) n_pos += alive[i];
        }
        const int32_t num_bg2 = par->rpn_batchsize - n_pos;
        if (!emit(f.n_low, f.n_low - num_bg2, f.n_low > num_bg2, &sz[2])) return MV3D_ERR_WORKSPACE;
        const int32_t fg_n = par->roi_fg_max < f.pt_n_fg ? par->roi_fg_max : f.pt_n_fg;
        if (!emit(f.pt_n_fg, fg_n, f.pt_n_fg > 0, &sz[3])) return MV3D_ERR_WORKSPACE;
        const int32_t bg_room = par->rois_per_image - fg_n;
        const int32_t bg_n = bg_room < f.pt_n_bg ? bg_room : f.pt_n_bg;
        if (!emit(f.pt_n_bg, bg_n < 0 ? 0 : bg_n, f.pt_n_bg > 0, &sz[4])) return MV3D_ERR_WORKSPACE;
    }
    return MV3D_OK;
}
```

### mv3d_tf_amd/csrc/train_stream.hip

```cpp
#include <hip/hip_runtime.h>
#include <chrono>
#include <condition_variable>
#include <deque>
#include <mutex>
#include <new>
#include <thread>
#include <vector>
#include "common.h"
#include "../../include/mv3d_hip.h"

#define TP_MAX_BATCH 16

namespace {

enum SlotState { TP_IDLE = 0, TP_SUBMITTED = 1, TP_STAGED = 2 };

struct Slot {
    mv3d_train_path_slot buf;
    hipEvent_t ev = nullptr;
    int state = TP_IDLE, rc = MV3D_OK;
    hipStream_t stream = nullptr;
    void *mt = nullptr;
    const float *calib = nullptr;
    const float *gt_bv[TP_MAX_BATCH], *gt_3d[TP_MAX_BATCH], *gt_c[TP_MAX_BATCH];
    int G[TP_MAX_BATCH];
    int32_t sizes[5 * TP_MAX_BATCH], rows[TP_MAX_BATCH];
    std::vector<uint8_t> spill[TP_MAX_BATCH];
    float *p_bv[TP_MAX_BATCH], *p_3d[TP_MAX_BATCH];
    int32_t *p_num[TP_MAX_BATCH], *p_cnt[TP_MAX_BATCH], *a_cnt[TP_MAX_BATCH];
    uint8_t *a_fgh[TP_MAX_BATCH];
    void *a_ws[TP_MAX_BATCH], *p_ws[TP_MAX_BATCH];
    int p_cap[TP_MAX_BATCH];
    size_t p_wsz[TP_MAX_BATCH];
    uint8_t *dv_report = nullptr;
    int32_t *dv_pt_counts = nullptr, *dv_num_proposals = nullptr;
};

static bool tp_force_copies()
{
#ifdef MV3D_TUNING
    return getenv("MV3D_TRAIN_PATH_COPIES") != nullptr;
#else
    return false;
#endif
}

__global__ __launch_bounds__(256) void tp_report_kernel(const uint8_t *__restrict__ report, size_t report_row, uint8_t *__restrict__ h_report,
                                                        size_t h_row, int B, const int32_t *__restrict__ pt_counts, int32_t *__restrict__ h_pt,
                                                        const int32_t *__restrict__ nump, int32_t *__restrict__ h_nump)
{
    const size_t v = h_row / 16;
    for (size_t i = threadIdx.x; i < (size_t)B * v; i += 256) {
        const size_t b = i / v, j = i - b * v;
        reinterpret_cast<uint4 *>(h_report + b * h_row)[j] = reinterpret_cast<const uint4 *>(report + b * report_row)[j];
    }
    for (int i = threadIdx.x; i < 4 * B; i += 256) h_pt[i] = pt_counts[i];
    for (int i = threadIdx.x; i < 2 * B; i += 256) h_nump[i] = nump[i];
}

}

struct mv3d_train_path {
    mv3d_train_path_config cfg;
    mv3d_proposal_target_params tpar[TP_MAX_BATCH];
    int depth = 0, device = 0;
    std::vector<Slot> slots;
    bool threaded = false, stop = false;
    std::thread helper;
    std::mutex m;
    std::condition_variable cv_work, cv_done;
    std::deque<int> queue;
    double t_wait = 0.0, t_draw = 0.0;
};

namespace {

bool config_ok(const mv3d_train_path_config &c)
{
    return c.batch >= 1 && c.batch <= TP_MAX_BATCH && c.H > 0 && c.W > 0 && c.num_classes >= 1 && c.proposal_cap > 0 && c.anchor_cap > 0 &&
           c.roi_cap > 0 && c.max_gt > 0 && c.draw.rois_per_image <= c.roi_cap;
}

void set_params(mv3d_train_path *tp, const mv3d_train_path_config &c)
{
    tp->cfg = c;
    for (int b = 0; b < c.batch; ++b) {
        tp->tpar[b] = c.target;
        tp->tpar[b].num_classes = c.num_classes;
        tp->tpar[b].frame_index = b;
    }
}

bool slot_ok(const mv3d_train_path_config &c, const mv3d_train_path_slot &s)
{
    const size_t N = (size_t)4 * c.H * c.W, B = (size_t)c.batch;
    if (!s.blob_bv || !s.blob_img || !s.blob_3d || !s.num_proposals || !s.proposal_ws || !s.rpn_labels || !s.rpn_targets || !s.anchors ||
        !s.anchors_3d || !s.n_anchors || !s.report || !s.pt_counts || !s.anchor_ws || !s.target_ws || !s.rois_bev || !s.rois_rgb ||
        !s.rois_3d || !s.labels || !s.bbox_targets || !s.lists || !s.h_report || !s.h_pt_counts || !s.h_num_proposals || !s.h_lists ||
        !s.h_scratch)
        return false;
    if (s.report_row % MV3D_ALIGN || s.report_row < 32 + N || s.h_report_row < 32 || s.h_report_row > s.report_row) return false;
    if (s.anchor_ws_bytes % MV3D_ALIGN || s.target_ws_bytes % MV3D_ALIGN) return false;
    if (s.lists_cap < B * (3 * N + 2 * ((size_t)c.proposal_cap + c.max_gt))) return false;
    if (s.scratch_cap < (N > (size_t)c.proposal_cap + c.max_gt ? N : (size_t)c.proposal_cap + c.max_gt)) return false;
    return true;
}

void slot_tables(const mv3d_train_path_config &c, Slot &s)
{
    const mv3d_train_path_slot &u = s.buf;
    for (int b = 0; b < c.batch; ++b) {
        s.p_bv[b] = u.blob_bv + (size_t)b * c.proposal_cap * 5;
        s.p_3d[b] = u.blob_3d + (size_t)b * c.proposal_cap * 7;
        s.p_num[b] = u.num_proposals + b;
        s.p_cnt[b] = u.pt_counts + 4 * b;
        s.a_cnt[b] = (int32_t *)(u.report + (size_t)b * u.report_row);
        s.a_fgh[b] = u.report + (size_t)b * u.report_row + 32;
        s.a_ws[b] = (char *)u.anchor_ws + (size_t)b * u.anchor_ws_bytes;
        s.p_ws[b] = (char *)u.target_ws + (size_t)b * u.target_ws_bytes;
        s.p_cap[b] = c.proposal_cap;
        s.p_wsz[b] = u.target_ws_bytes;
    }
}

#define TP_HIP(expr)                                 \
    do {                                             \
        if ((expr) != hipSuccess) return MV3D_ERR_HIP; \
    } while (0)

int host_stage(mv3d_train_path *tp, Slot &s)
{
    const mv3d_train_path_config &c = tp->cfg;
    const mv3d_train_path_slot &u = s.buf;
    const int B = c.batch, H = c.H, W = c.W;
    const auto t0 = std::chrono::steady_clock::now();
    TP_HIP(hipEventSynchronize(s.ev));
    const auto t1 = std::chrono::steady_clock::now();
    for (int b = 0; b < B; ++b)
        if (u.h_num_proposals[B + b] & MV3D_FLAG_ZERO_DIVISION) return MV3D_ERR_ZERO_DIVISION;
    mv3d_draw_frame fr[TP_MAX_BATCH];
    for (int b = 0; b < B; ++b) {
        const uint8_t *head = u.h_report + (size_t)b * u.h_report_row;
        const int32_t *cnt = (const int32_t *)head;
        fr[b].n_fg = cnt[1]; fr[b].n_bg = cnt[2]; fr[b].n_low = cnt[3];
        fr[b].pt_n_fg = u.h_pt_counts[4 * b + 1]; fr[b].pt_n_bg = u.h_pt_counts[4 * b + 2];
        fr[b].reserved0 = 0;
        if (cnt[1] < 0 || (size_t)cnt[1] > (size_t)4 * H * W) return MV3D_ERR_INVALID_ARG;
        if (32 + (size_t)cnt[1] <= u.h_report_row) {
            fr[b].fg_alive = head + 32;
        } else {
            s.spill[b].resize((size_t)cnt[1]);
            TP_HIP(hipMemcpyAsync(s.spill[b].data(), s.a_fgh[b], (size_t)cnt[1], hipMemcpyDeviceToHost, s.stream));
            TP_HIP(hipStreamSynchronize(s.stream));
            fr[b].fg_alive = s.spill[b].data();
        }
    }
    int rc = mv3d_draw_training_subsamples(s.mt, B, fr, &c.draw, u.h_lists, u.lists_cap, s.sizes, u.h_scratch, u.scratch_cap);
    const auto t2 = std::chrono::steady_clock::now();
    {
        std::lock_guard<std::mutex> g(tp->m);
        tp->t_wait += std::chrono::duration<double>(t1 - t0).count();
        tp->t_draw += std::chrono::duration<double>(t2 - t1).count();
    }
    if (rc != MV3D_OK) return rc;
    size_t off[5 * TP_MAX_BATCH + 1];
    off[0] = 0;
    for (int k = 0; k < 5 * B; ++k) off[k + 1] = off[k] + (size_t)s.sizes[k];
    const int32_t *const lists = u.lists;
    if (off[5 * B]) TP_HIP(hipMemcpyAsync(u.lists, u.h_lists, off[5 * B] * sizeof(int32_t), hipMemcpyHostToDevice, s.stream));
    const int32_t *lst[5][TP_MAX_BATCH];
    int cnt[5][TP_MAX_BATCH];
    for (int b = 0; b < B; ++b)
        for (int k = 0; k < 5; ++k) {
            cnt[k][b] = s.sizes[5 * b + k];
            lst[k][b] = cnt[k][b] ? lists + off[5 * b + k] : nullptr;
        }
    rc = mv3d_anchor_target_stage2_batch(B, H, W, &c.anchor, lst[0], cnt[0], lst[1], cnt[1], lst[2], cnt[2], u.rpn_labels, u.anchors,
                                         u.anchors_3d, u.n_anchors, c.anchor_cap, s.a_ws, u.anchor_ws_bytes, s.stream);
    if (rc != MV3D_OK) return rc;
    float *o_bev[TP_MAX_BATCH], *o_rgb[TP_MAX_BATCH], *o_fv[TP_MAX_BATCH], *o_3d[TP_MAX_BATCH], *o_tg[TP_MAX_BATCH];
    int32_t *o_lab[TP_MAX_BATCH];
    const float *cal[TP_MAX_BATCH];
    size_t row = 0;
    for (int b = 0; b < B; ++b) {
        const int S = cnt[3][b] + cnt[4][b];
        s.rows[b] = S;
        if (row + (size_t)S > (size_t)B * c.roi_cap) return MV3D_ERR_WORKSPACE;
        o_bev[b] = S ? u.rois_bev + row * 5 : nullptr;
        o_rgb[b] = S ? u.rois_rgb + row * 5 : nullptr;
        o_fv[b] = (S && u.rois_fv) ? u.rois_fv + row * 5 : nullptr;
        o_3d[b] = S ? u.rois_3d + row * 7 : nullptr;
        o_lab[b] = S ? u.labels + row : nullptr;
        o_tg[b] = S ? u.bbox_targets + row * 24 * c.num_classes : nullptr;
        cal[b] = s.calib + (size_t)b * 48;
        row += (size_t)S;
    }
    return mv3d_proposal_target_stage2_batch_devn(B, s.p_bv, s.p_3d, s.p_cap, s.p_num, s.gt_bv, s.gt_3d, s.gt_c, s.G, cal, tp->tpar, lst[3],
                                                  cnt[3], lst[4], cnt[4], o_bev, o_rgb, o_lab, o_tg, o_3d, u.rois_fv ? o_fv : nullptr, s.p_ws,
                                                  s.p_wsz, s.stream);
}

int host_stage_noexcept(mv3d_train_path *tp, Slot &s)
{
    try {
        return host_stage(tp, s);
    } catch (...) {
        return MV3D_ERR_WORKSPACE;
    }
}

void helper_main(mv3d_train_path *tp)
{
    (void)hipSetDevice(tp->device);
    for (;;) {
        int k;
        {
            std::unique_lock<std::mutex> g(tp->m);
            tp->cv_work.wait(g, [&] { return tp->stop || !tp->queue.empty(); });
            if (tp->queue.empty()) return;
            k = tp->queue.front();
            tp->queue.pop_front();
        }
        Slot &s = tp->slots[k];
        const int rc = host_stage_noexcept(tp, s);
        {
            std::lock_guard<std::mutex> g(tp->m);
            s.rc = rc;
            s.state = TP_STAGED;
        }
        tp->cv_done.notify_all();
    }
}

}

extern "C" int mv3d_train_path_create(const mv3d_train_path_config *config, int depth, const mv3d_train_path_slot *slots, int helper_thread,
                                      mv3d_train_path **out)
{
    if (!config || !slots || !out || depth < 1 || depth > 64 || !config_ok(*config)) return MV3D_ERR_INVALID_ARG;
    for (int k = 0; k < depth; ++k)
        if (!slot_ok(*config, slots[k])) return MV3D_ERR_INVALID_ARG;
    mv3d_train_path *tp = new (std::nothrow) mv3d_train_path();
    if (!tp) return MV3D_ERR_HIP;
    set_params(tp, *config);
    tp->depth = depth;
    if (hipGetDevice(&tp->device) != hipSuccess) { delete tp; return MV3D_ERR_HIP; }
    try {
        tp->slots.resize((size_t)depth);
    } catch (...) {
        delete tp;
        return MV3D_ERR_HIP;
    }
    for (int k = 0; k < depth; ++k) {
        Slot &s = tp->slots[k];
        s.buf = slots[k];
        slot_tables(tp->cfg, s);
        {
            void *d0 = nullptr, *d1 = nullptr, *d2 = nullptr;
            const bool mapped = hipHostGetDevicePointer(&d0, s.buf.h_report, 0) == hipSuccess && hipHostGetDevicePointer(&d1, s.buf.h_pt_counts, 0) == hipSuccess &&
                                hipHostGetDevicePointer(&d2, s.buf.h_num_proposals, 0) == hipSuccess && d0 && d1 && d2;
            (void)hipGetLastError();
            if (mapped && s.buf.h_report_row % 16 == 0 && (uintptr_t)d0 % 16 == 0 && (uintptr_t)s.buf.report % 16 == 0 && !tp_force_copies()) {
                s.dv_report = (uint8_t *)d0; s.dv_pt_counts = (int32_t *)d1; s.dv_num_proposals = (int32_t *)d2;
            }
        }
        if (hipEventCreateWithFlags(&s.ev, hipEventDisableTiming | hipEventBlockingSync) != hipSuccess) {
            for (int j = 0; j < k; ++j) (void)hipEventDestroy(tp->slots[j].ev);
            delete tp;
            return MV3D_ERR_HIP;
        }
    }
    tp->threaded = helper_thread != 0;
    if (tp->threaded) {
        try {
            tp->helper = std::thread(helper_main, tp);
        } catch (...) {
            for (Slot &s : tp->slots) (void)hipEventDestroy(s.ev);
            delete tp;
            return MV3D_ERR_HIP;
        }
    }
    *out = tp;
    return MV3D_OK;
}

extern "C" int mv3d_train_path_configure(mv3d_train_path *tp, const mv3d_train_path_config *c)
{
    if (!tp || !c || !config_ok(*c)) return MV3D_ERR_INVALID_ARG;
    const mv3d_train_path_config &o = tp->cfg;
    if (c->batch != o.batch || c->H != o.H || c->W != o.W || c->num_classes != o.num_classes || c->proposal_cap != o.proposal_cap ||
        c->anchor_cap != o.anchor_cap || c->roi_cap != o.roi_cap || c->max_gt != o.max_gt)
        return MV3D_ERR_INVALID_ARG;
    std::lock_guard<std::mutex> g(tp->m);
    for (const Slot &s : tp->slots)
        if (s.state != TP_IDLE) return MV3D_ERR_INVALID_ARG;
    set_params(tp, *c);
    return MV3D_OK;
}

extern "C" int mv3d_train_path_submit_masked(mv3d_train_path *tp, int slot, const float *prob, const float *pred, const float *im_info,
                                             const float *calib, const float *const *gt_bv, const float *const *gt_3d,
                                             const float *const *gt_corners, const int *G, const uint8_t *anchor_mask,
                                             void *mt19937_state, void *stream)
{
    if (!tp || slot < 0 || slot >= tp->depth || !prob || !pred || !im_info || !calib || !gt_bv || !gt_3d || !gt_corners || !G ||
        !mt19937_state)
        return MV3D_ERR_INVALID_ARG;
    const mv3d_train_path_config &c = tp->cfg;
    const int B = c.batch;
    for (int b = 0; b < B; ++b)
        if (G[b] < 1 || G[b] > c.max_gt || !gt_bv[b] || !gt_3d[b] || !gt_corners[b]) return MV3D_ERR_INVALID_ARG;
    Slot &s = tp->slots[slot];
    {
        std::lock_guard<std::mutex> g(tp->m);
        if (s.state != TP_IDLE) return MV3D_ERR_INVALID_ARG;
    }
    const mv3d_train_path_slot &u = s.buf;
    s.stream = (hipStream_t)stream;
    s.mt = mt19937_state;
    s.calib = calib;
    for (int b = 0; b < B; ++b) { s.gt_bv[b] = gt_bv[b]; s.gt_3d[b] = gt_3d[b]; s.gt_c[b] = gt_corners[b]; s.G[b] = G[b]; }
    const uint8_t *masks[TP_MAX_BATCH];
    for (int b = 0; b < B; ++b) masks[b] = anchor_mask ? anchor_mask + (size_t)b * 4 * c.H * c.W : nullptr;
    int rc = mv3d_proposal_3d_masked(prob, pred, B, c.H, c.W, im_info, calib, &c.proposal, anchor_mask, u.blob_bv, u.blob_img, u.blob_3d,
                                     u.num_proposals, u.num_proposals + B, u.proposal_ws, u.proposal_ws_bytes, stream);
    if (rc != MV3D_OK) return rc;
    rc = mv3d_anchor_target_stage1_batch_masked(B, c.H, c.W, im_info, s.gt_bv, s.gt_3d, s.G, &c.anchor, masks, u.rpn_labels, u.rpn_targets,
                                                s.a_cnt, s.a_fgh, s.a_ws, u.anchor_ws_bytes, stream);
    if (rc != MV3D_OK) return rc;
    rc = mv3d_proposal_target_stage1_batch_devn(B, s.p_bv, s.p_3d, s.p_cap, s.p_num, s.gt_bv, s.gt_3d, s.G, tp->tpar, s.p_cnt, s.p_ws,
                                                s.p_wsz, stream);
    if (rc != MV3D_OK) return rc;
    if (s.dv_report) {
        hipLaunchKernelGGL(tp_report_kernel, dim3(1), dim3(256), 0, s.stream, (const uint8_t *)u.report, (size_t)u.report_row, s.dv_report,
                           (size_t)u.h_report_row, B, (const int32_t *)u.pt_counts, s.dv_pt_counts, (const int32_t *)u.num_proposals,
                           s.dv_num_proposals);
        if (mv3d_launch_status() != MV3D_OK) return MV3D_ERR_HIP;
    } else {
        TP_HIP(hipMemcpy2DAsync(u.h_report, u.h_report_row, u.report, u.report_row, u.h_report_row, (size_t)B, hipMemcpyDeviceToHost, s.stream));
        TP_HIP(hipMemcpyAsync(u.h_pt_counts, u.pt_counts, (size_t)B * 4 * sizeof(int32_t), hipMemcpyDeviceToHost, s.stream));
        TP_HIP(hipMemcpyAsync(u.h_num_proposals, u.num_proposals, (size_t)B * 2 * sizeof(int32_t), hipMemcpyDeviceToHost, s.stream));
    }
    TP_HIP(hipEventRecord(s.ev, s.stream));
    {
        std::lock_guard<std::mutex> g(tp->m);
        s.state = TP_SUBMITTED;
        s.rc = MV3D_OK;
        if (tp->threaded) {
            try {
                tp->queue.push_back(slot);
            } catch (...) {
                s.state = TP_IDLE;
                return MV3D_ERR_HIP;
            }
        }
    }
    if (tp->threaded) tp->cv_work.notify_one();
    return MV3D_OK;
}

extern "C" int mv3d_train_path_submit(mv3d_train_path *tp, int slot, const float *prob, const float *pred, const float *im_info,
                                      const float *calib, const float *const *gt_bv, const float *const *gt_3d,
                                      const float *const *gt_corners, const int *G, void *mt19937_state, void *stream)
{
    return mv3d_train_path_submit_masked(tp, slot, prob, pred, im_info, calib, gt_bv, gt_3d, gt_corners, G, nullptr, mt19937_state, stream);
}

extern "C" int mv3d_train_path_finish(mv3d_train_path *tp, int slot, int32_t *rows_out, int32_t *num_proposals_out, int32_t *sizes_out)
{
    if (!tp || slot < 0 || slot >= tp->depth || !rows_out || !num_proposals_out) return MV3D_ERR_INVALID_ARG;
    Slot &s = tp->slots[slot];
    int rc;
    if (tp->threaded) {
        std::unique_lock<std::mutex> g(tp->m);
        if (s.state == TP_IDLE) return MV3D_ERR_INVALID_ARG;
        tp->cv_done.wait(g, [&] { return s.state == TP_STAGED; });
        rc = s.rc;
    } else {
        {
            std::lock_guard<std::mutex> g(tp->m);
            if (s.state != TP_SUBMITTED) return MV3D_ERR_INVALID_ARG;
        }
        rc = host_stage_noexcept(tp, s);
    }
    const int B = tp->cfg.batch;
    if (rc == MV3D_OK) {
        for (int b = 0; b < B; ++b) { rows_out[b] = s.rows[b]; num_proposals_out[b] = s.buf.h_num_proposals[b]; }
        if (sizes_out)
            for (int k = 0; k < 5 * B; ++k) sizes_out[k] = s.sizes[k];
    }
    std::lock_guard<std::mutex> g(tp->m);
    s.state = TP_IDLE;
    return rc;
}

extern "C" int mv3d_train_path_host_seconds(mv3d_train_path *tp, double *wait_s, double *draw_s)
{
    if (!tp) return MV3D_ERR_INVALID_ARG;
    std::lock_guard<std::mutex> g(tp->m);
    if (wait_s) *wait_s = tp->t_wait;
    if (draw_s) *draw_s = tp->t_draw;
    tp->t_wait = tp->t_draw = 0.0;
    return MV3D_OK;
}

extern "C" void mv3d_train_path_destroy(mv3d_train_path *tp)
{
    if (!tp) return;
    if (tp->threaded) {
        {
            std::lock_guard<std::mutex> g(tp->m);
            tp->stop = true;
        }
        tp->cv_work.notify_all();
        tp->helper.join();
    }
    for (Slot &s : tp->slots)
        if (s.ev) (void)hipEventDestroy(s.ev);
    delete tp;
}
```

### mv3d_tf_amd/train_path.py

```python
import ctypes as C

import numpy as np
import torch

from . import ops
from ._lib import DrawParams, TrainPathConfig, TrainPathSlot, check, lib
from .fast_rcnn.config import cfg
from .rpn_msr.anchor_target_layer_tf import REPORT_HEAD as _HEAD

def _global_mt19937_address():
    bg = np.random.mtrand._rand._bit_generator
    if not isinstance(bg, np.random.MT19937):
        raise TypeError("TrainPathStream draws on numpy's global legacy MT19937; the global bit generator is a %s" % type(bg).__name__)
    return bg.ctypes.state_address


class _Slot:
    pass


class TrainPathStream:

    def __init__(self, B, H, W, device, num_classes=2, depth=2, max_gt=64, want_fv=True, stream=None, async_draws=True, streams=None):
        self.B, self.H, self.W, self.dev, self.nc = int(B), int(H), int(W), torch.device(device), int(num_classes)
        self.N = self.H * self.W * 4
        self.want_fv = bool(want_fv)
        self.stream = stream
        self.streams = list(streams) if streams else None
        self.max_gt = int(max_gt)
        T = cfg.TRAIN
        self.anchor_cap = ops.anchor_debug_rows(T)
        self.roi_cap = int(T.BATCH_SIZE)
        L = lib()
        self.pparams = ops.proposal_params(T)
        self.cap = L.mv3d_proposal_3d_capacity(self.H, self.W, C.byref(self.pparams))
        if self.cap < 0:
            check(1, "mv3d_proposal_3d_capacity")
        self._cfg_key, self._config = self._make_config()
        self.slots = [self._make_slot(k) for k in range(int(depth))]
        for k, sl_ in enumerate(self.slots):
            sl_.stream = self.streams[k % len(self.streams)] if self.streams else self.stream
        self._slots_c = (TrainPathSlot * len(self.slots))(*[sl_.c for sl_ in self.slots])
        self._h = C.c_void_p()
        self.async_draws = bool(async_draws)
        with torch.cuda.device(self.dev):
            check(L.mv3d_train_path_create(C.byref(self._config), len(self.slots), self._slots_c, 1 if self.async_draws else 0,
                                           C.byref(self._h)), "mv3d_train_path_create")
        self._next = 0

    def _make_config(self):
        T = cfg.TRAIN
        rois_per_image = int(T.BATCH_SIZE) // 1
        key = (float(T.FG_THRESH), float(T.BG_THRESH_HI), float(T.BG_THRESH_LO), int(T.RPN_BATCHSIZE), float(T.RPN_FG_FRACTION),
               float(T.FG_FRACTION), rois_per_image, bool(T.RPN_CLOBBER_POSITIVES), float(T.RPN_NEGATIVE_OVERLAP), float(T.RPN_POSITIVE_OVERLAP))
        c = TrainPathConfig()
        c.batch, c.H, c.W, c.num_classes = self.B, self.H, self.W, self.nc
        c.proposal_cap, c.anchor_cap, c.roi_cap, c.max_gt = self.cap, self.anchor_cap, self.roi_cap, self.max_gt
        c.proposal = self.pparams
        c.anchor = ops.anchor_target_params(T)
        c.target = ops.proposal_target_params(T, self.nc)
        c.draw = DrawParams(int(T.RPN_BATCHSIZE), int(T.RPN_FG_FRACTION * T.RPN_BATCHSIZE), rois_per_image,
                            int(np.round(T.FG_FRACTION * rois_per_image)))
        return key, c

    def _make_slot(self, index):
        B, H, W, N, dev, nc, L = self.B, self.H, self.W, self.N, self.dev, self.nc, lib()
        s = _Slot()
        s.index = index
        e = lambda shape, dt=torch.float32: torch.empty(shape, dtype=dt, device=dev)
        s.pack, s.prop = ops.proposal_3d_outputs(B, self.cap, dev)
        s.tail = s.pack[s.pack.numel() - 2 * B:].view(torch.int32)
        s.pws = e((max(L.mv3d_proposal_3d_workspace_bytes(B, H, W, C.byref(self.pparams)), 256),), torch.uint8)
        s.rpn_labels, s.rpn_targets = e((B, N)), e((B, N, 6))
        s.anchors, s.anchors_3d = e((B, self.anchor_cap, 5)), e((B, self.anchor_cap, 7))
        s.n_anchors = e((B,), torch.int32)
        s.row = (32 + N + 255) // 256 * 256
        s.report = e((B, s.row), torch.uint8)
        s.pt_counts = e((B, 4), torch.int32)
        s.awsz = (max(L.mv3d_anchor_target_workspace_bytes(H, W, self.max_gt), 256) + 255) // 256 * 256
        s.aws = e((B, s.awsz), torch.uint8)
        s.twsz = (max(L.mv3d_proposal_target_workspace_bytes(self.cap, self.max_gt), 256) + 255) // 256 * 256
        s.tws = e((B, s.twsz), torch.uint8)
        S = B * self.roi_cap
        s.rois = {"bev": e((S, 5)), "rgb": e((S, 5)), "fv": e((S, 5))}
        s.rois_3d, s.labels, s.bbox_targets = e((S, 7)), e((S, 1), torch.int32), e((S, 24 * nc))
        head = min(_HEAD, s.row)
        s.h_report = torch.empty((B, head), dtype=torch.uint8).pin_memory()
        s.h_small = torch.empty((B, 4), dtype=torch.int32).pin_memory()
        s.h_tail = torch.empty((2 * B,), dtype=torch.int32).pin_memory()
        s.list_cap = B * (3 * N + 2 * (self.cap + self.max_gt))
        s.h_lists = torch.empty((s.list_cap,), dtype=torch.int32).pin_memory()
        s.h_scratch = torch.empty((max(N, self.cap + self.max_gt) + 64,), dtype=torch.int32)
        s.d_lists = e((s.list_cap,), torch.int32)
        bv, img, b3, num, status = s.prop
        assert s.tail.data_ptr() == num.data_ptr() and status.data_ptr() == num.data_ptr() + 4 * B
        c = s.c = TrainPathSlot()
        c.blob_bv, c.blob_img, c.blob_3d, c.num_proposals = bv.data_ptr(), img.data_ptr(), b3.data_ptr(), s.tail.data_ptr()
        c.proposal_ws, c.proposal_ws_bytes = s.pws.data_ptr(), s.pws.numel()
        c.rpn_labels, c.rpn_targets, c.anchors, c.anchors_3d = (t.data_ptr() for t in (s.rpn_labels, s.rpn_targets, s.anchors, s.anchors_3d))
        c.n_anchors, c.report, c.report_row, c.pt_counts = s.n_anchors.data_ptr(), s.report.data_ptr(), s.row, s.pt_counts.data_ptr()
        c.anchor_ws, c.anchor_ws_bytes, c.target_ws, c.target_ws_bytes = s.aws.data_ptr(), s.awsz, s.tws.data_ptr(), s.twsz
        c.rois_bev, c.rois_rgb = s.rois["bev"].data_ptr(), s.rois["rgb"].data_ptr()
        c.rois_fv = s.rois["fv"].data_ptr() if self.want_fv else None
        c.rois_3d, c.labels, c.bbox_targets = s.rois_3d.data_ptr(), s.labels.data_ptr(), s.bbox_targets.data_ptr()
        c.lists, c.lists_cap = s.d_lists.data_ptr(), s.list_cap
        c.h_report, c.h_report_row, c.h_pt_counts, c.h_num_proposals = s.h_report.data_ptr(), head, s.h_small.data_ptr(), s.h_tail.data_ptr()
        c.h_lists, c.h_scratch, c.scratch_cap = s.h_lists.data_ptr(), s.h_scratch.data_ptr(), s.h_scratch.numel()
        s.rows_c, s.nprop_c, s.sizes_c = (C.c_int32 * B)(), (C.c_int32 * B)(), (C.c_int32 * (5 * B))()
        s.busy = False
        return s

    def submit(self, prob, pred, im_info, calib, gt, anchor_mask=None):
        B, L = self.B, lib()
        s = self.slots[self._next]
        if s.busy:
            raise RuntimeError("TrainPathStream: every slot is in flight (finish() one first, or raise `depth`)")
        G = [int(g[0].shape[0]) for g in gt]
        if len(G) != B or max(G) > self.max_gt or min(G) <= 0:
            raise ValueError("TrainPathStream: %d frames with 1 .. max_gt = %d ground-truth boxes each, got %s" % (B, self.max_gt, G))
        key, conf = self._make_config()
        if key != self._cfg_key:
            if any(sl_.busy for sl_ in self.slots):
                raise RuntimeError("TrainPathStream: cfg.TRAIN changed while a batch is in flight")
            check(L.mv3d_train_path_configure(self._h, C.byref(conf)), "mv3d_train_path_configure")
            self._cfg_key, self._config = key, conf
        self._next = (self._next + 1) % len(self.slots)
        mask = ops.anchor_mask_tensor(anchor_mask, B, self.N, self.dev)
        if s.stream is not None:
            s.stream.wait_stream(torch.cuda.current_stream())
        st = (s.stream or torch.cuda.current_stream()).cuda_stream
        s.inputs = (prob, pred, im_info, calib, gt, mask)
        s.G = G
        mt = _global_mt19937_address()
        PP = C.c_void_p * B
        ptrs = (PP(*[g[0].data_ptr() for g in gt]), PP(*[g[1].data_ptr() for g in gt]), PP(*[g[2].data_ptr() for g in gt]), (C.c_int * B)(*G))
        if mask is None:
            check(L.mv3d_train_path_submit(self._h, s.index, prob.data_ptr(), pred.data_ptr(), im_info.data_ptr(), calib.data_ptr(),
                                           *ptrs, mt, st), "mv3d_train_path_submit")
        else:
            check(L.mv3d_train_path_submit_masked(self._h, s.index, prob.data_ptr(), pred.data_ptr(), im_info.data_ptr(), calib.data_ptr(),
                                                  *ptrs, mask.data_ptr(), mt, st), "mv3d_train_path_submit_masked")
        s.busy = True
        return s

    def close(self):
        h, self._h = getattr(self, "_h", None), None
        if h:
            lib().mv3d_train_path_destroy(h)

    def __del__(self):
        try:
            self.close()
        except Exception:
            pass

    @property
    def host_seconds(self):
        w, d = C.c_double(), C.c_double()
        check(lib().mv3d_train_path_host_seconds(self._h, C.byref(w), C.byref(d)), "mv3d_train_path_host_seconds")
        return w.value, d.value

    def finish(self, s):
        s.busy = False
        check(lib().mv3d_train_path_finish(self._h, s.index, s.rows_c, s.nprop_c, s.sizes_c), "mv3d_train_path_finish")
        S = list(s.rows_c)
        St = sum(S)
        return {"rpn_labels": s.rpn_labels, "rpn_targets": s.rpn_targets, "anchors": s.anchors, "anchors_3d": s.anchors_3d,
                "n_anchors": s.n_anchors, "rois": {k: v[:St] for k, v in s.rois.items()}, "rois_3d": s.rois_3d[:St],
                "labels": s.labels[:St], "bbox_targets": s.bbox_targets[:St], "S": S,
                "num_proposals": list(s.nprop_c), "proposals": s.prop, "stream": s.stream, "draw_sizes": list(s.sizes_c)}
```

Baseline: 17030.

## Emit kept-bitmasks from host subsample draw and vectorize MT19937 permutation

The host-side training subsample draw now yields a per-frame bitmask of kept anchors instead of full disable-index lists. A persistent identity buffer is used so the permutation only shuffles the needed tail, and the Mersenne Twister generation, tempering and bounded-rejection scan are vectorized with AVX2 clones. A new stage-2 kernel reads the bitmasks to disable the non-kept fg/bg/low anchors. The aim is to cut host draw time and the host-to-device list copy. The cost is extra code paths plus profiling counters and timing calls added to the enqueue path.

```diff
diff --git a/include/mv3d_hip.h b/include/mv3d_hip.h
--- a/include/mv3d_hip.h
+++ b/include/mv3d_hip.h
@@ -167,6 +167,12 @@
                                     const int32_t *const *disable_bg2_dev, const int *n_dis_bg2, float *labels_dev,
                                     float *anchors_dev, float *anchors_3d_dev, int32_t *n_anchors_dev, int anchors_cap,
                                     void *const *workspace, size_t workspace_bytes, void *stream);
+int mv3d_anchor_target_stage2_batch_kept(int batch, int H, int W, const mv3d_anchor_target_params *p,
+                                         const uint32_t *const *kept_fg_dev, const int *n_fg,
+                                         const uint32_t *const *kept_bg_dev, const int *n_bg,
+                                         const uint32_t *const *kept_low_dev, const int *n_low, float *labels_dev,
+                                         float *anchors_dev, float *anchors_3d_dev, int32_t *n_anchors_dev, int anchors_cap,
+                                         void *const *workspace, size_t workspace_bytes, void *stream);
 
 typedef struct {
     int32_t num_classes;
@@ -262,6 +268,9 @@
 } mv3d_draw_params;
 int mv3d_draw_training_subsamples(void *mt19937_state, int batch, const mv3d_draw_frame *frames, const mv3d_draw_params *par,
                                   int32_t *lists, size_t lists_cap, int32_t *sizes, int32_t *scratch, size_t scratch_cap);
+int mv3d_draw_training_subsamples_kept(void *mt19937_state, int batch, const mv3d_draw_frame *frames, const mv3d_draw_params *par,
+                                       int32_t *lists, size_t lists_cap, int32_t *sizes, int32_t *scratch, size_t scratch_cap,
+                                       int32_t *ident, size_t ident_cap);
 
 typedef struct {
     int32_t batch, H, W, num_classes;
@@ -307,6 +316,7 @@
                                   const uint8_t *anchor_mask_dev, void *mt19937_state, void *stream);
 int mv3d_train_path_finish(mv3d_train_path *path, int slot, int32_t *rows_out, int32_t *num_proposals_out, int32_t *sizes_out);
 int mv3d_train_path_host_seconds(mv3d_train_path *path, double *wait_s, double *draw_s);
+int mv3d_train_path_host_profile(mv3d_train_path *path, double *seconds, int64_t *batches);
 void mv3d_train_path_destroy(mv3d_train_path *path);
 
 int mv3d_gt_encode(const float *box_cam_dev, const double *cos_sin_dev, int num_objects, const float *inv_rot_dev,
diff --git a/mv3d_tf_amd/_lib.py b/mv3d_tf_amd/_lib.py
--- a/mv3d_tf_amd/_lib.py
+++ b/mv3d_tf_amd/_lib.py
@@ -162,6 +162,8 @@
                                                          _P, _P, _P, _P, C.c_size_t, _P]),
     "mv3d_anchor_target_stage2_batch": (C.c_int, [C.c_int, C.c_int, C.c_int, C.POINTER(AnchorTargetParams), _P, _P, _P, _P, _P, _P, _P,
                                                   _P, _P, _P, C.c_int, _P, C.c_size_t, _P]),
+    "mv3d_anchor_target_stage2_batch_kept": (C.c_int, [C.c_int, C.c_int, C.c_int, C.POINTER(AnchorTargetParams), _P, _P, _P, _P, _P, _P,
+                                                       _P, _P, _P, _P, C.c_int, _P, C.c_size_t, _P]),
     "mv3d_proposal_target_stage1_batch": (C.c_int, [C.c_int, _P, _P, _P, _P, _P, _P, _P, _P, _P, _P, _P]),
     "mv3d_proposal_target_stage2_batch": (C.c_int, [C.c_int, _P, _P, _P, _P, _P, _P, _P, _P, _P, _P, _P, _P, _P, _P, _P, _P, _P, _P, _P,
                                                     _P, _P, _P]),
@@ -217,12 +219,15 @@
     "mv3d_legacy_permutation": (C.c_int, [_P, C.c_int32, _P]),
     "mv3d_draw_training_subsamples": (C.c_int, [_P, C.c_int, C.POINTER(DrawFrame), C.POINTER(DrawParams), _P, C.c_size_t, _P, _P,
                                                 C.c_size_t]),
+    "mv3d_draw_training_subsamples_kept": (C.c_int, [_P, C.c_int, C.POINTER(DrawFrame), C.POINTER(DrawParams), _P, C.c_size_t, _P, _P,
+                                                     C.c_size_t, _P, C.c_size_t]),
     "mv3d_train_path_create": (C.c_int, [C.POINTER(TrainPathConfig), C.c_int, C.POINTER(TrainPathSlot), C.c_int, C.POINTER(C.c_void_p)]),
     "mv3d_train_path_configure": (C.c_int, [_P, C.POINTER(TrainPathConfig)]),
     "mv3d_train_path_submit": (C.c_int, [_P, C.c_int, _P, _P, _P, _P, _P, _P, _P, _P, _P, _P]),
     "mv3d_train_path_submit_masked": (C.c_int, [_P, C.c_int, _P, _P, _P, _P, _P, _P, _P, _P, _P, _P, _P]),
     "mv3d_train_path_finish": (C.c_int, [_P, C.c_int, _P, _P, _P]),
     "mv3d_train_path_host_seconds": (C.c_int, [_P, C.POINTER(C.c_double), C.POINTER(C.c_double)]),
+    "mv3d_train_path_host_profile": (C.c_int, [_P, C.POINTER(C.c_double), C.POINTER(C.c_int64)]),
     "mv3d_train_path_destroy": (None, [_P]),
     "mv3d_gt_encode": (C.c_int, [_P, _P, C.c_int, _P, _P, _P, _P, _P, _P, _P]),
     "mv3d_conv3x3_f16": (C.c_int, [_P, _P, _P, _P, C.c_int, C.c_int, C.c_int, C.c_int, C.c_int, C.c_int, C.c_int, C.c_int, _P]),
diff --git a/mv3d_tf_amd/csrc/anchor_target.hip b/mv3d_tf_amd/csrc/anchor_target.hip
--- a/mv3d_tf_amd/csrc/anchor_target.hip
+++ b/mv3d_tf_amd/csrc/anchor_target.hip
@@ -175,6 +175,23 @@
     }
 }
 
+__global__ __launch_bounds__(256) void at_disable_kept_kernel(AtBatch bt)
+{
+    const AtFrame &F = bt.f[blockIdx.y];
+    const int n1 = F.n_dis_fg, n2 = F.n_dis_bg1, n3 = F.n_dis_bg2;
+    const unsigned N = (unsigned)F.d.N;
+    for (int t = blockIdx.x * blockDim.x + threadIdx.x; t < n1 + n2 + n3; t += gridDim.x * blockDim.x) {
+        const int k = t < n1 ? 0 : (t < n1 + n2 ? 1 : 2);
+        const int p = t - (k == 0 ? 0 : (k == 1 ? n1 : n1 + n2));
+        const uint32_t *kept = reinterpret_cast<const uint32_t *>(k == 0 ? F.dis_fg : (k == 1 ? F.dis_bg1 : F.dis_bg2));
+        if ((kept[p >> 5] >> (p & 31)) & 1u) continue;
+        const unsigned a = (unsigned)(k == 0 ? F.lists.fg : (k == 1 ? F.lists.bg : F.lists.low))[p];
+        if (a >= N) continue;
+        if (k == 2) F.d.argmax[a] = -1;
+        else F.d.labels[a] = -1.0f;
+    }
+}
+
 __global__ __launch_bounds__(256) void at_emit_relabel_kernel(AtBatch bt)
 {
     const AtFrame &F = bt.f[blockIdx.y];
@@ -303,12 +320,12 @@
                                            &counts_dev, &fg_hi_dev, &workspace, workspace_bytes, stream);
 }
 
-extern "C" int mv3d_anchor_target_stage2_batch(int batch, int H, int W, const mv3d_anchor_target_params *p,
-                                               const int32_t *const *disable_fg_dev, const int *n_dis_fg,
-                                               const int32_t *const *disable_bg1_dev, const int *n_dis_bg1,
-                                               const int32_t *const *disable_bg2_dev, const int *n_dis_bg2, float *labels_dev,
-                                               float *anchors_dev, float *anchors_3d_dev, int32_t *n_anchors_dev,
-                                               int anchors_cap, void *const *workspace, size_t workspace_bytes, void *stream)
+static int at_stage2(bool kept, int batch, int H, int W, const mv3d_anchor_target_params *p,
+                     const int32_t *const *disable_fg_dev, const int *n_dis_fg,
+                     const int32_t *const *disable_bg1_dev, const int *n_dis_bg1,
+                     const int32_t *const *disable_bg2_dev, const int *n_dis_bg2, float *labels_dev,
+                     float *anchors_dev, float *anchors_3d_dev, int32_t *n_anchors_dev,
+                     int anchors_cap, void *const *workspace, size_t workspace_bytes, void *stream)
 {
     if (batch <= 0 || batch > AT_MAX_BATCH || !p || !labels_dev || !workspace || !n_dis_fg || !n_dis_bg1 || !n_dis_bg2 ||
         !disable_fg_dev || !disable_bg1_dev || !disable_bg2_dev)
@@ -321,7 +338,8 @@
     int most = 0;
     for (int b = 0; b < batch; ++b) {
         if (n_dis_fg[b] < 0 || n_dis_bg1[b] < 0 || n_dis_bg2[b] < 0) return MV3D_ERR_INVALID_ARG;
-        if ((n_dis_fg[b] && !disable_fg_dev[b]) || (n_dis_bg1[b] && !disable_bg1_dev[b]) || (n_dis_bg2[b] && !disable_bg2_dev[b]))
+        if (kept && (n_dis_fg[b] > L.N || n_dis_bg1[b] > L.N || n_dis_bg2[b] > L.N)) return MV3D_ERR_INVALID_ARG;
+        if (!kept && ((n_dis_fg[b] && !disable_fg_dev[b]) || (n_dis_bg1[b] && !disable_bg1_dev[b]) || (n_dis_bg2[b] && !disable_bg2_dev[b])))
             return MV3D_ERR_INVALID_ARG;
         if (!workspace[b] || workspace_bytes < L.total || ((uintptr_t)workspace[b] % MV3D_ALIGN)) return MV3D_ERR_WORKSPACE;
         AtFrame &F = bt.f[b];
@@ -330,16 +348,45 @@
         F.d.labels = labels_dev + (size_t)b * L.N;
         F.dis_fg = disable_fg_dev[b]; F.dis_bg1 = disable_bg1_dev[b]; F.dis_bg2 = disable_bg2_dev[b];
         F.n_dis_fg = n_dis_fg[b]; F.n_dis_bg1 = n_dis_bg1[b]; F.n_dis_bg2 = n_dis_bg2[b];
+        if (kept) {
+            if (!F.dis_fg) F.n_dis_fg = 0;
+            if (!F.dis_bg1) F.n_dis_bg1 = 0;
+            if (!F.dis_bg2) F.n_dis_bg2 = 0;
+        }
         F.anchors = emit ? anchors_dev + (size_t)b * anchors_cap * 5 : nullptr;
         F.anchors_3d = emit ? anchors_3d_dev + (size_t)b * anchors_cap * 7 : nullptr;
         F.n_anchors = emit ? n_anchors_dev + b : nullptr;
-        const int n = n_dis_fg[b] + n_dis_bg1[b] + n_dis_bg2[b];
+        const int n = F.n_dis_fg + F.n_dis_bg1 + F.n_dis_bg2;
         if (n > most) most = n;
     }
     hipStream_t s = (hipStream_t)stream;
-    if (most > 0) hipLaunchKernelGGL(at_disable_all_kernel, dim3((most + 255) / 256, batch), dim3(256), 0, s, bt);
+    if (most > 0 && kept) hipLaunchKernelGGL(at_disable_kept_kernel, dim3((most + 255) / 256, batch), dim3(256), 0, s, bt);
+    else if (most > 0) hipLaunchKernelGGL(at_disable_all_kernel, dim3((most + 255) / 256, batch), dim3(256), 0, s, bt);
     hipLaunchKernelGGL(at_emit_relabel_kernel, dim3(L.ncwg, batch), dim3(256), 0, s, bt);
     return mv3d_launch_status();
+}
+
+extern "C" int mv3d_anchor_target_stage2_batch(int batch, int H, int W, const mv3d_anchor_target_params *p,
+                                               const int32_t *const *disable_fg_dev, const int *n_dis_fg,
+                                               const int32_t *const *disable_bg1_dev, const int *n_dis_bg1,
+                                               const int32_t *const *disable_bg2_dev, const int *n_dis_bg2, float *labels_dev,
+                                               float *anchors_dev, float *anchors_3d_dev, int32_t *n_anchors_dev,
+                                               int anchors_cap, void *const *workspace, size_t workspace_bytes, void *stream)
+{
+    return at_stage2(false, batch, H, W, p, disable_fg_dev, n_dis_fg, disable_bg1_dev, n_dis_bg1, disable_bg2_dev, n_dis_bg2, labels_dev,
+                     anchors_dev, anchors_3d_dev, n_anchors_dev, anchors_cap, workspace, workspace_bytes, stream);
+}
+
+extern "C" int mv3d_anchor_target_stage2_batch_kept(int batch, int H, int W, const mv3d_anchor_target_params *p,
+                                                    const uint32_t *const *kept_fg_dev, const int *n_fg,
+                                                    const uint32_t *const *kept_bg_dev, const int *n_bg,
+                                                    const uint32_t *const *kept_low_dev, const int *n_low, float *labels_dev,
+                                                    float *anchors_dev, float *anchors_3d_dev, int32_t *n_anchors_dev,
+                                                    int anchors_cap, void *const *workspace, size_t workspace_bytes, void *stream)
+{
+    return at_stage2(true, batch, H, W, p, reinterpret_cast<const int32_t *const *>(kept_fg_dev), n_fg,
+                     reinterpret_cast<const int32_t *const *>(kept_bg_dev), n_bg, reinterpret_cast<const int32_t *const *>(kept_low_dev), n_low,
+                     labels_dev, anchors_dev, anchors_3d_dev, n_anchors_dev, anchors_cap, workspace, workspace_bytes, stream);
 }
 
 extern "C" int mv3d_anchor_target_stage2(int H, int W, const mv3d_anchor_target_params *p,
diff --git a/mv3d_tf_amd/csrc/legacy_rng.hip b/mv3d_tf_amd/csrc/legacy_rng.hip
--- a/mv3d_tf_amd/csrc/legacy_rng.hip
+++ b/mv3d_tf_amd/csrc/legacy_rng.hip
@@ -7,22 +7,102 @@
 constexpr int MT_N = 624, MT_M = 397;
 struct MtState { uint32_t key[MT_N]; int pos; };
 
-inline void mt_gen(MtState *s)
-{
-    uint32_t *k = s->key;
-    int i;
-    for (i = 0; i < MT_N - MT_M; ++i) {
+#if defined(__x86_64__) && !defined(__HIP_DEVICE_COMPILE__) && !defined(MV3D_NO_SIMD_CLONES)
+#define MV3D_X86_CLONES 1
+#define MV3D_AVX2 __attribute__((target("avx2")))
+#endif
+#define MV3D_SIMD_BODY static inline __attribute__((always_inline))
+
+#define MT_TWIST(y) (((y) >> 1) ^ ((0u - ((y) & 1u)) & 0x9908b0dfu))
+MV3D_SIMD_BODY void mt_gen_body(MtState *s)
+{
+    uint32_t *__restrict__ k = s->key;
+#pragma clang loop vectorize(enable) interleave(enable)
+    for (int i = 0; i < MT_N - MT_M; ++i) {
         const uint32_t y = (k[i] & 0x80000000u) | (k[i + 1] & 0x7fffffffu);
-        k[i] = k[i + MT_M] ^ (y >> 1) ^ ((y & 1u) ? 0x9908b0dfu : 0u);
-    }
-    for (; i < MT_N - 1; ++i) {
+        k[i] = k[i + MT_M] ^ MT_TWIST(y);
+    }
+#pragma clang loop vectorize(enable) interleave(enable)
+    for (int i = MT_N - MT_M; i < MT_N - 1; ++i) {
         const uint32_t y = (k[i] & 0x80000000u) | (k[i + 1] & 0x7fffffffu);
-        k[i] = k[i + (MT_M - MT_N)] ^ (y >> 1) ^ ((y & 1u) ? 0x9908b0dfu : 0u);
+        k[i] = k[i + (MT_M - MT_N)] ^ MT_TWIST(y);
     }
     const uint32_t y = (k[MT_N - 1] & 0x80000000u) | (k[0] & 0x7fffffffu);
-    k[MT_N - 1] = k[MT_M - 1] ^ (y >> 1) ^ ((y & 1u) ? 0x9908b0dfu : 0u);
+    k[MT_N - 1] = k[MT_M - 1] ^ MT_TWIST(y);
     s->pos = 0;
 }
+
+MV3D_SIMD_BODY void temper_body(const uint32_t *__restrict__ key, uint32_t *__restrict__ t, int from)
+{
+#pragma clang loop vectorize(enable)
+    for (int k = from; k < MT_N; ++k) {
+        uint32_t y = key[k];
+        y ^= (y >> 11);
+        y ^= (y << 7) & 0x9d2c5680u;
+        y ^= (y << 15) & 0xefc60000u;
+        y ^= (y >> 18);
+        t[k] = y;
+    }
+}
+
+template <int B>
+MV3D_SIMD_BODY int32_t scan_count_body(const uint32_t *__restrict__ t, uint32_t mask, int32_t i, int32_t *amb)
+{
+    const int32_t sure = i - B;
+    int32_t a = 0, b = 0;
+#pragma clang loop vectorize(enable)
+    for (int k = 0; k < B; ++k) {
+        const int32_t w = (int32_t)(t[k] & mask);
+        a += (w <= sure) ? 1 : 0;
+        b += (w <= i) ? 1 : 0;
+    }
+    *amb = b - a;
+    return a;
+}
+
+MV3D_SIMD_BODY int32_t scan_body(const uint32_t *__restrict__ t, int *pos_io, int32_t i, int32_t lo, uint32_t mask)
+{
+    int pos = *pos_io;
+    while (pos + 32 <= MT_N && i - 32 > lo) {
+        int32_t amb;
+        const int32_t acc = scan_count_body<32>(t + pos, mask, i, &amb);
+        if (!amb) { i -= acc; pos += 32; continue; }
+        for (int q = 0; q < 4; ++q, pos += 8) {
+            const int32_t acc8 = scan_count_body<8>(t + pos, mask, i, &amb);
+            if (!amb) { i -= acc8; continue; }
+            for (int k = 0; k < 8; ++k) i -= ((t[pos + k] & mask) <= (uint32_t)i) ? 1 : 0;
+        }
+    }
+    while (pos < MT_N && i > lo) i -= ((t[pos++] & mask) <= (uint32_t)i) ? 1 : 0;
+    *pos_io = pos;
+    return i;
+}
+
+struct SimdOps {
+    void (*gen)(MtState *);
+    void (*temper)(const uint32_t *, uint32_t *, int);
+    int32_t (*scan)(const uint32_t *, int *, int32_t, int32_t, uint32_t);
+};
+void gen_base(MtState *s) { mt_gen_body(s); }
+void temper_base(const uint32_t *key, uint32_t *t, int from) { temper_body(key, t, from); }
+int32_t scan_base(const uint32_t *t, int *pos, int32_t i, int32_t lo, uint32_t mask) { return scan_body(t, pos, i, lo, mask); }
+#ifdef MV3D_X86_CLONES
+MV3D_AVX2 void gen_avx2(MtState *s) { mt_gen_body(s); }
+MV3D_AVX2 void temper_avx2(const uint32_t *key, uint32_t *t, int from) { temper_body(key, t, from); }
+MV3D_AVX2 int32_t scan_avx2(const uint32_t *t, int *pos, int32_t i, int32_t lo, uint32_t mask) { return scan_body(t, pos, i, lo, mask); }
+#endif
+const SimdOps &simd_ops()
+{
+    static const SimdOps ops = [] {
+#ifdef MV3D_X86_CLONES
+        if (__builtin_cpu_supports("avx2")) return SimdOps{gen_avx2, temper_avx2, scan_avx2};
+#endif
+        return SimdOps{gen_base, temper_base, scan_base};
+    }();
+    return ops;
+}
+
+inline void mt_gen(MtState *s) { mt_gen_body(s); }
 
 inline uint32_t mt_next(MtState *s)
 {
@@ -71,6 +151,42 @@
     s->pos = pos;
 }
 
+void permutation_tail(MtState *s, int32_t n, int32_t K, int32_t *out, int32_t *ident, int32_t *touched)
+{
+    const SimdOps &ops = simd_ops();
+    const int32_t first = n - K < 1 ? 1 : n - K;
+    int32_t i = n - 1, nt = 0;
+    int pos = s->pos;
+    uint32_t t[MT_N];
+    int t_lo = MT_N;
+    while (i >= 1) {
+        const uint32_t mask = 0xffffffffu >> __builtin_clz((uint32_t)i);
+        const int32_t lo = (int32_t)(mask >> 1);
+        while (i > lo) {
+            if (pos == MT_N) { ops.gen(s); pos = 0; t_lo = MT_N; }
+            if (t_lo > pos) { ops.temper(s->key, t, pos); t_lo = pos; }
+            if (i >= first) {
+                const int32_t end = lo > first - 1 ? lo : first - 1;
+                while (pos < MT_N && i > end) {
+                    const uint32_t j = t[pos++] & mask;
+                    if (j <= (uint32_t)i) {
+                        const int32_t a = ident[i], b = ident[j];
+                        ident[i] = b; ident[j] = a;
+                        touched[nt++] = (int32_t)j;
+                        --i;
+                    }
+                }
+                continue;
+            }
+            i = ops.scan(t, &pos, i, lo, mask);
+        }
+    }
+    s->pos = pos;
+    for (int32_t k = 0; k < K; ++k) out[k] = ident[n - K + k];
+    for (int32_t k = n - K; k < n; ++k) ident[k] = k;
+    for (int32_t k = 0; k < nt; ++k) ident[touched[k]] = touched[k];
+}
+
 }
 
 extern "C" int mv3d_legacy_permutation(void *mt19937_state, int32_t n, int32_t *out)
@@ -132,3 +248,73 @@
     }
     return MV3D_OK;
 }
+
+extern "C" int mv3d_draw_training_subsamples_kept(void *mt19937_state, int batch, const mv3d_draw_frame *frames,
+                                                  const mv3d_draw_params *par, int32_t *lists, size_t lists_cap, int32_t *sizes,
+                                                  int32_t *scratch, size_t scratch_cap, int32_t *ident, size_t ident_cap)
+{
+    if (!mt19937_state || batch <= 0 || !frames || !par || !lists || !sizes || !scratch) return MV3D_ERR_INVALID_ARG;
+    MtState *s = (MtState *)mt19937_state;
+    if (s->pos < 0 || s->pos > MT_N) return MV3D_ERR_INVALID_ARG;
+    size_t o = 0;
+    int rc = MV3D_OK;
+    auto emit_kept = [&](int32_t n, int32_t keep, bool draw, int32_t *size_out, const uint32_t **bits_out) -> bool {
+        *size_out = 0;
+        *bits_out = nullptr;
+        if (!draw) return true;
+        const size_t words = ((size_t)(n < 0 ? 0 : n) + 31) / 32;
+        if (n < 0 || keep < 0 || keep > n || o + words > lists_cap) return false;
+        const int32_t *tail;
+        if (ident && (size_t)n <= ident_cap && 2 * (size_t)keep <= scratch_cap) {
+            permutation_tail(s, n, keep, scratch, ident, scratch + keep);
+            tail = scratch;
+        } else {
+            if ((size_t)n > scratch_cap) return false;
+            permutation(s, n, scratch);
+            tail = scratch + (n - keep);
+        }
+        uint32_t *bits = (uint32_t *)(lists + o);
+        memset(bits, 0, words * sizeof(uint32_t));
+        for (int32_t k = 0; k < keep; ++k) {
+            const uint32_t v = (uint32_t)tail[k];
+            if (v >= (uint32_t)n) { rc = MV3D_ERR_INVALID_ARG; return false; }
+            bits[v >> 5] |= 1u << (v & 31);
+        }
+        *size_out = n - keep;
+        *bits_out = bits;
+        o += words;
+        return true;
+    };
+    auto emit = [&](int32_t n, int32_t take, bool draw, int32_t *size_out) -> bool {
+        *size_out = 0;
+        if (!draw) return true;
+        if (n < 0 || (size_t)n > scratch_cap || take < 0 || take > n || o + (size_t)take > lists_cap) return false;
+        permutation(s, n, scratch);
+        memcpy(lists + o, scratch, (size_t)take * sizeof(int32_t));
+        *size_out = take;
+        o += (size_t)take;
+        return true;
+    };
+    for (int b = 0; b < batch; ++b) {
+        const mv3d_draw_frame &f = frames[b];
+        int32_t *sz = sizes + 5 * b;
+        if (f.n_fg < 0 || f.n_bg < 0 || f.n_low < 0 || f.pt_n_fg < 0 || f.pt_n_bg < 0 || (f.n_fg > 0 && !f.fg_alive))
+            return MV3D_ERR_INVALID_ARG;
+        const uint32_t *kept_fg, *unused;
+        const int32_t num_fg = par->rpn_num_fg;
+        if (!emit_kept(f.n_fg, num_fg, f.n_fg > num_fg, &sz[0], &kept_fg)) return rc != MV3D_OK ? rc : MV3D_ERR_WORKSPACE;
+        const int32_t num_bg = par->rpn_batchsize - (f.n_fg < num_fg ? f.n_fg : num_fg);
+        if (!emit_kept(f.n_bg, num_bg, f.n_bg > num_bg, &sz[1], &unused)) return rc != MV3D_OK ? rc : MV3D_ERR_WORKSPACE;
+        int32_t n_pos = 0;
+        for (int32_t i = 0; i < f.n_fg; ++i)
+            n_pos += (f.fg_alive[i] && (!kept_fg || ((kept_fg[i >> 5] >> (i & 31)) & 1u))) ? 1 : 0;
+        const int32_t num_bg2 = par->rpn_batchsize - n_pos;
+        if (!emit_kept(f.n_low, num_bg2, f.n_low > num_bg2, &sz[2], &unused)) return rc != MV3D_OK ? rc : MV3D_ERR_WORKSPACE;
+        const int32_t fg_n = par->roi_fg_max < f.pt_n_fg ? par->roi_fg_max : f.pt_n_fg;
+        if (!emit(f.pt_n_fg, fg_n, f.pt_n_fg > 0, &sz[3])) return MV3D_ERR_WORKSPACE;
+        const int32_t bg_room = par->rois_per_image - fg_n;
+        const int32_t bg_n = bg_room < f.pt_n_bg ? bg_room : f.pt_n_bg;
+        if (!emit(f.pt_n_bg, bg_n < 0 ? 0 : bg_n, f.pt_n_bg > 0, &sz[4])) return MV3D_ERR_WORKSPACE;
+    }
+    return MV3D_OK;
+}
diff --git a/mv3d_tf_amd/csrc/train_stream.hip b/mv3d_tf_amd/csrc/train_stream.hip
--- a/mv3d_tf_amd/csrc/train_stream.hip
+++ b/mv3d_tf_amd/csrc/train_stream.hip
@@ -71,6 +71,9 @@
     std::condition_variable cv_work, cv_done;
     std::deque<int> queue;
     double t_wait = 0.0, t_draw = 0.0;
+    double prof[4] = {0.0, 0.0, 0.0, 0.0};
+    long long prof_batches = 0;
+    std::vector<int32_t> ident;
 };
 
 namespace {
@@ -101,7 +104,7 @@
         return false;
     if (s.report_row % MV3D_ALIGN || s.report_row < 32 + N || s.h_report_row < 32 || s.h_report_row > s.report_row) return false;
     if (s.anchor_ws_bytes % MV3D_ALIGN || s.target_ws_bytes % MV3D_ALIGN) return false;
-    if (s.lists_cap < B * (3 * N + 2 * ((size_t)c.proposal_cap + c.max_gt))) return false;
+    if (s.lists_cap < B * (3 * ((N + 31) / 32) + 2 * ((size_t)c.proposal_cap + c.max_gt))) return false;
     if (s.scratch_cap < (N > (size_t)c.proposal_cap + c.max_gt ? N : (size_t)c.proposal_cap + c.max_gt)) return false;
     return true;
 }
@@ -155,28 +158,41 @@
             fr[b].fg_alive = s.spill[b].data();
         }
     }
-    int rc = mv3d_draw_training_subsamples(s.mt, B, fr, &c.draw, u.h_lists, u.lists_cap, s.sizes, u.h_scratch, u.scratch_cap);
+    int rc = mv3d_draw_training_subsamples_kept(s.mt, B, fr, &c.draw, u.h_lists, u.lists_cap, s.sizes, u.h_scratch, u.scratch_cap,
+                                                tp->ident.data(), tp->ident.size());
     const auto t2 = std::chrono::steady_clock::now();
     {
         std::lock_guard<std::mutex> g(tp->m);
         tp->t_wait += std::chrono::duration<double>(t1 - t0).count();
         tp->t_draw += std::chrono::duration<double>(t2 - t1).count();
+        tp->prof[0] += std::chrono::duration<double>(t1 - t0).count();
+        tp->prof[1] += std::chrono::duration<double>(t2 - t1).count();
     }
     if (rc != MV3D_OK) return rc;
     size_t off[5 * TP_MAX_BATCH + 1];
     off[0] = 0;
-    for (int k = 0; k < 5 * B; ++k) off[k + 1] = off[k] + (size_t)s.sizes[k];
+    for (int b = 0; b < B; ++b) {
+        const int32_t n[3] = {fr[b].n_fg, fr[b].n_bg, fr[b].n_low};
+        for (int k = 0; k < 5; ++k) {
+            const int32_t sz = s.sizes[5 * b + k];
+            off[5 * b + k + 1] = off[5 * b + k] + (k < 3 ? (sz > 0 ? ((size_t)n[k] + 31) / 32 : 0) : (size_t)sz);
+        }
+    }
     const int32_t *const lists = u.lists;
     if (off[5 * B]) TP_HIP(hipMemcpyAsync(u.lists, u.h_lists, off[5 * B] * sizeof(int32_t), hipMemcpyHostToDevice, s.stream));
     const int32_t *lst[5][TP_MAX_BATCH];
     int cnt[5][TP_MAX_BATCH];
-    for (int b = 0; b < B; ++b)
+    for (int b = 0; b < B; ++b) {
+        const int32_t n[3] = {fr[b].n_fg, fr[b].n_bg, fr[b].n_low};
         for (int k = 0; k < 5; ++k) {
-            cnt[k][b] = s.sizes[5 * b + k];
-            lst[k][b] = cnt[k][b] ? lists + off[5 * b + k] : nullptr;
-        }
-    rc = mv3d_anchor_target_stage2_batch(B, H, W, &c.anchor, lst[0], cnt[0], lst[1], cnt[1], lst[2], cnt[2], u.rpn_labels, u.anchors,
-                                         u.anchors_3d, u.n_anchors, c.anchor_cap, s.a_ws, u.anchor_ws_bytes, s.stream);
+            const bool any = off[5 * b + k + 1] > off[5 * b + k];
+            cnt[k][b] = k < 3 ? (any ? n[k] : 0) : s.sizes[5 * b + k];
+            lst[k][b] = any ? lists + off[5 * b + k] : nullptr;
+        }
+    }
+    rc = mv3d_anchor_target_stage2_batch_kept(B, H, W, &c.anchor, (const uint32_t *const *)lst[0], cnt[0], (const uint32_t *const *)lst[1], cnt[1],
+                                              (const uint32_t *const *)lst[2], cnt[2], u.rpn_labels, u.anchors, u.anchors_3d, u.n_anchors,
+                                              c.anchor_cap, s.a_ws, u.anchor_ws_bytes, s.stream);
     if (rc != MV3D_OK) return rc;
     float *o_bev[TP_MAX_BATCH], *o_rgb[TP_MAX_BATCH], *o_fv[TP_MAX_BATCH], *o_3d[TP_MAX_BATCH], *o_tg[TP_MAX_BATCH];
     int32_t *o_lab[TP_MAX_BATCH];
@@ -195,9 +211,16 @@
         cal[b] = s.calib + (size_t)b * 48;
         row += (size_t)S;
     }
-    return mv3d_proposal_target_stage2_batch_devn(B, s.p_bv, s.p_3d, s.p_cap, s.p_num, s.gt_bv, s.gt_3d, s.gt_c, s.G, cal, tp->tpar, lst[3],
-                                                  cnt[3], lst[4], cnt[4], o_bev, o_rgb, o_lab, o_tg, o_3d, u.rois_fv ? o_fv : nullptr, s.p_ws,
-                                                  s.p_wsz, s.stream);
+    rc = mv3d_proposal_target_stage2_batch_devn(B, s.p_bv, s.p_3d, s.p_cap, s.p_num, s.gt_bv, s.gt_3d, s.gt_c, s.G, cal, tp->tpar, lst[3],
+                                                cnt[3], lst[4], cnt[4], o_bev, o_rgb, o_lab, o_tg, o_3d, u.rois_fv ? o_fv : nullptr, s.p_ws,
+                                                s.p_wsz, s.stream);
+    const auto t3 = std::chrono::steady_clock::now();
+    {
+        std::lock_guard<std::mutex> g(tp->m);
+        tp->prof[2] += std::chrono::duration<double>(t3 - t2).count();
+        tp->prof_batches += 1;
+    }
+    return rc;
 }
 
 int host_stage_noexcept(mv3d_train_path *tp, Slot &s)
@@ -216,7 +239,11 @@
         int k;
         {
             std::unique_lock<std::mutex> g(tp->m);
-            tp->cv_work.wait(g, [&] { return tp->stop || !tp->queue.empty(); });
+            if (!tp->stop && tp->queue.empty()) {
+                const auto i0 = std::chrono::steady_clock::now();
+                tp->cv_work.wait(g, [&] { return tp->stop || !tp->queue.empty(); });
+                tp->prof[3] += std::chrono::duration<double>(std::chrono::steady_clock::now() - i0).count();
+            }
             if (tp->queue.empty()) return;
             k = tp->queue.front();
             tp->queue.pop_front();
@@ -247,6 +274,8 @@
     if (hipGetDevice(&tp->device) != hipSuccess) { delete tp; return MV3D_ERR_HIP; }
     try {
         tp->slots.resize((size_t)depth);
+        tp->ident.resize((size_t)4 * config->H * config->W);
+        for (size_t v = 0; v < tp->ident.size(); ++v) tp->ident[v] = (int32_t)v;
     } catch (...) {
         delete tp;
         return MV3D_ERR_HIP;
@@ -404,6 +433,16 @@
     return MV3D_OK;
 }
 
+extern "C" int mv3d_train_path_host_profile(mv3d_train_path *tp, double *seconds, int64_t *batches)
+{
+    if (!tp) return MV3D_ERR_INVALID_ARG;
+    std::lock_guard<std::mutex> g(tp->m);
+    if (seconds)
+        for (int k = 0; k < 4; ++k) seconds[k] = tp->prof[k];
+    if (batches) *batches = (int64_t)tp->prof_batches;
+    return MV3D_OK;
+}
+
 extern "C" void mv3d_train_path_destroy(mv3d_train_path *tp)
 {
     if (!tp) return;
diff --git a/mv3d_tf_amd/train_path.py b/mv3d_tf_amd/train_path.py
--- a/mv3d_tf_amd/train_path.py
+++ b/mv3d_tf_amd/train_path.py
@@ -160,6 +160,12 @@
         check(lib().mv3d_train_path_host_seconds(self._h, C.byref(w), C.byref(d)), "mv3d_train_path_host_seconds")
         return w.value, d.value
 
+    @property
+    def host_profile(self):
+        sec, n = (C.c_double * 4)(), C.c_int64()
+        check(lib().mv3d_train_path_host_profile(self._h, sec, C.byref(n)), "mv3d_train_path_host_profile")
+        return dict(zip(("wait", "draw", "enqueue", "idle"), sec)), n.value
+
     def finish(self, s):
         s.busy = False
         check(lib().mv3d_train_path_finish(self._h, s.index, s.rows_c, s.nprop_c, s.sizes_c), "mv3d_train_path_finish")
```

Result: no change. 16920 (-0.6%).
